# 2235854410/CCVPE

Hardware: AMD Instinct MI355X
Metric: query images/sec (VIGOR, 512x512 sat / 320x640 grd) (higher is better)
Workload: dtype f32; 1 GPU; vigor_samearea_fov360_b32; variant=vigor_ori_prior, batch_per_gpu=32, global_batch=32, parallelism=image-parallel x1, all_gather of 20 B/query results, schedule=two streams per GPU (aerial encoder + orientation decoder on the second)

## Files before the change

ccvpe_amd/_lib.py:

```python
from __future__ import annotations

import ctypes as C
import os

_HERE = os.path.dirname(os.path.abspath(__file__))
LIB_PATH = os.path.join(_HERE, "csrc", "libccvpe_hip.so")

OK = 0
VARIANT_ID = {"vigor": 0, "vigor_ori_prior": 1, "kitti": 2, "oxford": 3}


class Config(C.Structure):
    _fields_ = [("variant", C.c_int32), ("circular_padding", C.c_int32), ("ori_noise", C.c_float),
                ("device", C.c_int32), ("micro_batch", C.c_int32), ("reserved", C.c_int32 * 3)]


class Outputs(C.Structure):
    _fields_ = [("logits_flattened", C.c_void_p), ("heatmap", C.c_void_p), ("ori", C.c_void_p),
                ("matching_score", C.c_void_p * 6)]


class Pose(C.Structure):
    _fields_ = [("index", C.c_int32), ("prob", C.c_float), ("cos_v", C.c_float), ("sin_v", C.c_float),
                ("angle_deg", C.c_float)]


SYMBOLS = [
    ("ccvpe_last_error", C.c_char_p, []),
    ("ccvpe_version", C.c_char_p, []),
    ("ccvpe_launch_count", C.c_uint64, []),
    ("ccvpe_create", C.c_int, [C.POINTER(Config), C.POINTER(C.c_void_p)]),
    ("ccvpe_destroy", C.c_int, [C.c_void_p]),
    ("ccvpe_set_weight", C.c_int, [C.c_void_p, C.c_char_p, C.c_void_p, C.POINTER(C.c_int64), C.c_int32]),
    ("ccvpe_skip_weight", C.c_int, [C.c_void_p, C.c_char_p]),
    ("ccvpe_finalize_weights", C.c_int, [C.c_void_p]),
    ("ccvpe_save_packed", C.c_int, [C.c_void_p, C.c_char_p]),
    ("ccvpe_load_packed", C.c_int, [C.c_void_p, C.c_char_p]),
    ("ccvpe_pack_switches", C.c_char_p, []),
    ("ccvpe_import_tuning", C.c_int, [C.c_void_p, C.c_char_p]),
    ("ccvpe_export_tuning", C.c_int, [C.c_void_p, C.c_char_p, C.c_size_t, C.POINTER(C.c_size_t)]),
    ("ccvpe_tuning_generation", C.c_int, [C.c_void_p]),
    ("ccvpe_max_micro_batch", C.c_int, [C.c_int32, C.c_float, C.c_int32, C.c_int32]),
    ("ccvpe_output_channels", C.c_int, [C.c_void_p, C.c_int32]),
    ("ccvpe_workspace_bytes", C.c_size_t, [C.c_void_p, C.c_int32, C.c_int32, C.c_int32]),
    ("ccvpe_forward", C.c_int, [C.c_void_p, C.c_void_p, C.c_int32, C.c_int32, C.c_void_p, C.c_int32,
                                C.POINTER(Outputs), C.c_void_p]),
    ("ccvpe_postprocess", C.c_int, [C.c_void_p, C.c_void_p, C.c_void_p, C.c_int32, C.c_void_p, C.c_void_p]),
    ("ccvpe_postprocess_rows", C.c_int, [C.c_void_p, C.c_void_p, C.c_void_p, C.c_int32, C.c_void_p, C.c_void_p]),
    ("ccvpe_postprocess_topk", C.c_int, [C.c_void_p, C.c_void_p, C.c_void_p, C.c_int32, C.c_int32, C.c_int32, C.c_void_p,
                                         C.c_void_p]),
    ("ccvpe_eval_metrics", C.c_int, [C.c_void_p, C.c_void_p, C.c_void_p, C.c_int32, C.c_void_p, C.c_void_p, C.c_void_p, C.c_void_p,
                                     C.c_void_p, C.c_void_p]),
    ("ccvpe_aerial_cache_bytes", C.c_size_t, [C.c_void_p, C.c_int32]),
    ("ccvpe_encode_aerial", C.c_int, [C.c_void_p, C.c_void_p, C.c_int32, C.c_void_p, C.c_void_p]),
    ("ccvpe_forward_cached", C.c_int, [C.c_void_p, C.c_void_p, C.c_int32, C.c_int32, C.c_void_p, C.c_int32,
                                       C.POINTER(Outputs), C.c_void_p]),
    ("ccvpe_localize", C.c_int, [C.c_void_p, C.c_void_p, C.c_int32, C.c_int32, C.c_void_p, C.c_int32, C.c_void_p, C.c_void_p]),
    ("ccvpe_localize_cached", C.c_int, [C.c_void_p, C.c_void_p, C.c_int32, C.c_int32, C.c_void_p, C.c_int32, C.c_void_p,
                                        C.c_void_p]),
    ("ccvpe_localize_topk", C.c_int, [C.c_void_p, C.c_void_p, C.c_int32, C.c_int32, C.c_void_p, C.c_int32, C.c_int32, C.c_int32,
                                      C.c_void_p, C.c_void_p]),
    ("ccvpe_localize_topk_cached", C.c_int, [C.c_void_p, C.c_void_p, C.c_int32, C.c_int32, C.c_void_p, C.c_int32, C.c_int32,
                                             C.c_int32, C.c_void_p, C.c_void_p]),
    ("ccvpe_forward_cached_indexed", C.c_int, [C.c_void_p, C.c_void_p, C.c_int32, C.c_int32, C.c_void_p, C.c_int32, C.c_void_p,
                                               C.c_int32, C.POINTER(Outputs), C.c_void_p]),
    ("ccvpe_localize_cached_indexed", C.c_int, [C.c_void_p, C.c_void_p, C.c_int32, C.c_int32, C.c_void_p, C.c_int32, C.c_void_p,
                                                C.c_int32, C.c_void_p, C.c_void_p]),
    ("ccvpe_localize_topk_cached_indexed", C.c_int, [C.c_void_p, C.c_void_p, C.c_int32, C.c_int32, C.c_void_p, C.c_int32, C.c_void_p,
                                                     C.c_int32, C.c_int32, C.c_int32, C.c_void_p, C.c_void_p]),
    ("ccvpe_ground_cache_bytes", C.c_size_t, [C.c_void_p, C.c_int32, C.c_int32, C.c_int32]),
    ("ccvpe_encode_ground", C.c_int, [C.c_void_p, C.c_void_p, C.c_int32, C.c_int32, C.c_int32, C.c_void_p, C.c_void_p]),
    ("ccvpe_localize_region", C.c_int, [C.c_void_p, C.c_void_p, C.c_int32, C.c_int32, C.c_int32, C.c_void_p, C.c_int32, C.c_void_p,
                                        C.c_void_p, C.c_void_p, C.c_void_p, C.c_void_p, C.c_void_p, C.c_void_p, C.c_void_p]),
    ("ccvpe_localize_prior", C.c_int, [C.c_void_p, C.c_void_p, C.c_int32, C.c_int32, C.c_void_p, C.c_int32, C.c_void_p, C.c_int64,
                                       C.c_int32, C.c_int32, C.c_void_p, C.c_void_p]),
    ("ccvpe_localize_prior_cached_indexed", C.c_int, [C.c_void_p, C.c_void_p, C.c_int32, C.c_int32, C.c_void_p, C.c_int32, C.c_void_p,
                                                      C.c_int32, C.c_void_p, C.c_int64, C.c_int32, C.c_int32, C.c_void_p, C.c_void_p]),
    ("ccvpe_postprocess_prior", C.c_int, [C.c_void_p, C.c_void_p, C.c_void_p, C.c_int32, C.c_void_p, C.c_int64, C.c_int32, C.c_int32,
                                          C.c_void_p, C.c_void_p]),
    ("ccvpe_localize_region_prior", C.c_int, [C.c_void_p, C.c_void_p, C.c_int32, C.c_int32, C.c_int32, C.c_void_p, C.c_int32, C.c_void_p,
                                              C.c_void_p, C.c_void_p, C.c_int64, C.c_void_p, C.c_void_p, C.c_void_p, C.c_void_p, C.c_void_p,
                                              C.c_void_p]),
    ("ccvpe_track_update", C.c_int, [C.c_void_p, C.c_void_p, C.c_int32, C.c_int32, C.c_void_p, C.c_int32, C.c_void_p, C.c_int64,
                                     C.c_void_p, C.c_void_p, C.c_void_p]),
    ("ccvpe_track_update_cached_indexed", C.c_int, [C.c_void_p, C.c_void_p, C.c_int32, C.c_int32, C.c_void_p, C.c_int32, C.c_void_p,
                                                    C.c_int32, C.c_void_p, C.c_int64, C.c_void_p, C.c_void_p, C.c_void_p]),
    ("ccvpe_track_update_logits", C.c_int, [C.c_void_p, C.c_void_p, C.c_void_p, C.c_int32, C.c_void_p, C.c_int64, C.c_void_p,
                                            C.c_void_p, C.c_void_p]),
    ("ccvpe_track_predict", C.c_int, [C.c_void_p, C.c_void_p, C.c_int32, C.c_void_p, C.c_void_p, C.c_int32, C.c_int32, C.c_void_p,
                                      C.c_void_p, C.c_void_p]),
    ("ccvpe_preprocess", C.c_int, [C.c_void_p, C.c_int32, C.c_int32, C.c_int32, C.c_void_p, C.c_int32,
                                   C.POINTER(C.c_float * 3), C.POINTER(C.c_float * 3), C.c_void_p, C.c_void_p]),
    ("ccvpe_preprocess_resize", C.c_int, [C.c_void_p, C.c_int32, C.c_int32, C.c_int32, C.c_int32, C.c_int32, C.c_void_p, C.c_int32,
                                          C.POINTER(C.c_float * 3), C.POINTER(C.c_float * 3), C.c_void_p, C.c_void_p, C.c_void_p]),
    ("ccvpe_preprocess_affine", C.c_int, [C.c_void_p, C.c_int32, C.c_int32, C.c_int32, C.c_void_p, C.POINTER(C.c_int32), C.c_int32,
                                          C.c_int32, C.c_int32, C.c_int32, C.c_int32, C.POINTER(C.c_float * 3), C.POINTER(C.c_float * 3),
                                          C.c_void_p, C.c_void_p]),
    ("ccvpe_preprocess_window_resize", C.c_int, [C.c_void_p, C.c_int32, C.c_int32, C.c_void_p, C.c_int32, C.c_int32, C.c_int32,
                                                 C.c_int32, C.c_int32, C.POINTER(C.c_float * 3), C.POINTER(C.c_float * 3), C.c_void_p,
                                                 C.c_void_p, C.c_void_p]),
    ("ccvpe_set_debug", C.c_int, [C.c_void_p, C.c_int32]),
    ("ccvpe_set_streams", C.c_int, [C.c_void_p, C.c_int32]),
    ("ccvpe_read_tap", C.c_int, [C.c_void_p, C.c_char_p, C.c_void_p, C.c_size_t, C.POINTER(C.c_size_t),
                                 C.POINTER(C.c_int32 * 4)]),
    ("ccvpe_debug_dump_plan", C.c_int, [C.c_void_p, C.c_char_p]),
    ("ccvpe_profile_forward", C.c_int, [C.c_void_p, C.c_void_p, C.c_int32, C.c_int32, C.c_void_p, C.c_int32,
                                        C.POINTER(Outputs), C.c_void_p]),
    ("ccvpe_profile_row", C.c_int, [C.c_void_p, C.c_int32, C.c_char_p, C.c_size_t, C.POINTER(C.c_float),
                                    C.POINTER(C.c_double), C.POINTER(C.c_double)]),
    ("ccvpe_profile_row_issued", C.c_int, [C.c_void_p, C.c_int32, C.POINTER(C.c_double)]),
    ("ccvpe_op_num_tiles", C.c_int, []),
    ("ccvpe_op_tile_name", C.c_char_p, [C.c_int32]),
    ("ccvpe_op_conv2d", C.c_int, [C.c_void_p, C.c_int32, C.c_int32, C.c_int32, C.c_int32, C.c_void_p, C.c_void_p,
                                  C.c_int32, C.c_int32, C.c_int32, C.c_int32, C.c_int32, C.c_int32, C.c_int32,
                                  C.c_void_p, C.c_int32, C.POINTER(C.c_float), C.c_void_p]),
]


IMAGENET_MEAN = (0.485, 0.456, 0.406)
IMAGENET_STD = (0.229, 0.224, 0.225)


def preprocess(img_u8_hwc, shift=None, crop_w=None, mean=IMAGENET_MEAN, std=IMAGENET_STD):
    import torch
    lib = load()
    assert img_u8_hwc.is_cuda and img_u8_hwc.dtype == torch.uint8 and img_u8_hwc.dim() == 4 and img_u8_hwc.shape[3] == 3
    img = img_u8_hwc.contiguous()
    B, H, W, _ = img.shape
    crop_w = W if crop_w is None else int(crop_w)
    out = torch.empty((B, 3, H, crop_w), dtype=torch.float32, device=img.device)
    sh = None
    if shift is not None:
        sh = torch.as_tensor(shift, dtype=torch.int32, device=img.device).contiguous()
        assert sh.numel() == B
    m = (C.c_float * 3)(*mean)
    s = (C.c_float * 3)(*std)
    stream = torch.cuda.current_stream(img.device).cuda_stream
    rc = lib.ccvpe_preprocess(C.c_void_p(img.data_ptr()), B, H, W, C.c_void_p(sh.data_ptr()) if sh is not None else None,
                              crop_w, C.byref(m), C.byref(s), C.c_void_p(out.data_ptr()), C.c_void_p(stream))
    check(rc, "ccvpe_preprocess")
    return out


def preprocess_resize(img_u8_hwc, out_hw, shift=None, crop_w=None, mean=IMAGENET_MEAN, std=IMAGENET_STD):
    import torch
    lib = load()
    assert img_u8_hwc.is_cuda and img_u8_hwc.dtype == torch.uint8 and img_u8_hwc.dim() == 4 and img_u8_hwc.shape[3] == 3
    img = img_u8_hwc.contiguous()
    B, H, W, _ = img.shape
    OH, OW = int(out_hw[0]), int(out_hw[1])
    crop_w = OW if crop_w is None else int(crop_w)
    out = torch.empty((B, 3, OH, crop_w), dtype=torch.float32, device=img.device)
    scratch = torch.empty((B, H, OW, 3), dtype=torch.uint8, device=img.device) if W != OW else None
    sh = None
    if shift is not None:
        sh = torch.as_tensor(shift, dtype=torch.int32, device=img.device).contiguous()
        assert sh.numel() == B
    m = (C.c_float * 3)(*mean)
    s = (C.c_float * 3)(*std)
    stream = torch.cuda.current_stream(img.device).cuda_stream
    rc = lib.ccvpe_preprocess_resize(C.c_void_p(img.data_ptr()), B, H, W, OH, OW, C.c_void_p(sh.data_ptr()) if sh is not None else None,
                                     crop_w, C.byref(m), C.byref(s), C.c_void_p(scratch.data_ptr()) if scratch is not None else None,
                                     C.c_void_p(out.data_ptr()), C.c_void_p(stream))
    check(rc, "ccvpe_preprocess_resize")
    return out


RESAMPLE = {"nearest": 0, "bilinear": 2}


def preprocess_affine(img_u8_hwc, matrices, filters, crop, mean=IMAGENET_MEAN, std=IMAGENET_STD):
    import torch
    lib = load()
    assert img_u8_hwc.is_cuda and img_u8_hwc.dtype == torch.uint8 and img_u8_hwc.dim() == 4 and img_u8_hwc.shape[3] == 3
    img = img_u8_hwc.contiguous()
    B, H, W, _ = img.shape
    mat = torch.as_tensor(matrices, dtype=torch.float64).to(img.device).contiguous()
    n = len(filters)
    assert mat.shape == (B, n, 6), (tuple(mat.shape), B, n)
    flt = (C.c_int32 * n)(*[RESAMPLE[f] if isinstance(f, str) else int(f) for f in filters])
    top, left, out_h, out_w = (int(v) for v in crop)
    out = torch.empty((B, 3, max(out_h, 0), max(out_w, 0)), dtype=torch.float32, device=img.device)
    m = (C.c_float * 3)(*mean)
    s = (C.c_float * 3)(*std)
    stream = torch.cuda.current_stream(img.device).cuda_stream
    rc = lib.ccvpe_preprocess_affine(C.c_void_p(img.data_ptr()), B, H, W, C.c_void_p(mat.data_ptr()), flt, n, top, left, out_h, out_w,
                                     C.byref(m), C.byref(s), C.c_void_p(out.data_ptr()), C.c_void_p(stream))
    check(rc, "ccvpe_preprocess_affine")
    return out


def preprocess_window_resize(map_u8_hwc, origins, win_hw, out_hw, mean=IMAGENET_MEAN, std=IMAGENET_STD):
    import torch
    lib = load()
    assert map_u8_hwc.is_cuda and map_u8_hwc.dtype == torch.uint8 and map_u8_hwc.dim() == 3 and map_u8_hwc.shape[2] == 3
    mp = map_u8_hwc.contiguous()
    org = torch.as_tensor(origins, dtype=torch.int32).reshape(-1, 2).to(mp.device).contiguous()
    B = org.shape[0]
    win_h, win_w = int(win_hw[0]), int(win_hw[1])
    out_h, out_w = int(out_hw[0]), int(out_hw[1])
    out = torch.empty((B, 3, max(out_h, 0), max(out_w, 0)), dtype=torch.float32, device=mp.device)
    scratch = torch.empty((max(B * win_h * out_w * 3, 1),), dtype=torch.uint8, device=mp.device)
    m = (C.c_float * 3)(*mean)
    s = (C.c_float * 3)(*std)
    stream = torch.cuda.current_stream(mp.device).cuda_stream
    rc = lib.ccvpe_preprocess_window_resize(C.c_void_p(mp.data_ptr()), mp.shape[0], mp.shape[1], C.c_void_p(org.data_ptr()), B, win_h, win_w,
                                            out_h, out_w, C.byref(m), C.byref(s), C.c_void_p(scratch.data_ptr()), C.c_void_p(out.data_ptr()),
                                            C.c_void_p(stream))
    check(rc, "ccvpe_preprocess_window_resize")
    return out


def op_conv2d(x_nhwc, w, bias=None, stride=1, pad=0, act=0, tile=0, iters=0):
    import torch
    lib = load()
    B, H, W, Cin = x_nhwc.shape
    Cout, _, KH, KW = w.shape
    OH = (H + 2 * pad - KH) // stride + 1
    OW = (W + 2 * pad - KW) // stride + 1
    out = torch.empty((B, OH, OW, Cout), dtype=torch.float32, device=x_nhwc.device)
    x_nhwc = x_nhwc.contiguous()
    w = w.contiguous().float()
    b = bias.contiguous().float() if bias is not None else None
    ms = C.c_float(0.0)
    stream = torch.cuda.current_stream(x_nhwc.device).cuda_stream
    rc = lib.ccvpe_op_conv2d(C.c_void_p(x_nhwc.data_ptr()), B, H, W, Cin, C.c_void_p(w.data_ptr()),
                             C.c_void_p(b.data_ptr()) if b is not None else None, Cout, KH, KW, stride, pad, act, tile,
                             C.c_void_p(out.data_ptr()), iters, C.byref(ms), C.c_void_p(stream))
    check(rc, "ccvpe_op_conv2d")
    return out, (ms.value if iters > 0 else None)

_lib = None


def library_digest() -> str:
    override = os.environ.get("CCVPE_LIB_PATH")
    if override:
        import hashlib
        h = hashlib.sha256()
        with open(override, "rb") as fh:
            for chunk in iter(lambda: fh.read(1 << 20), b""):
                h.update(chunk)
        return h.hexdigest()
    from . import build as _build
    return _build._digest()


def load() -> C.CDLL:
    global _lib
    if _lib is not None:
        return _lib
    try:
        import torch
    except ImportError:
        pass
    override = os.environ.get("CCVPE_LIB_PATH")
    if override:
        lib = C.CDLL(override)
        for name, res, args in SYMBOLS:
            fn = getattr(lib, name)
            fn.restype = res
            fn.argtypes = args
        _lib = lib
        return lib
    try:
        from . import build as _build
        if not _build.is_current():
            _build.build(verbose=False)
    except Exception as e:
        if os.path.exists(LIB_PATH):
            import warnings
            warnings.warn(f"libccvpe_hip.so may be stale and could not be rebuilt: {e}")
    if not os.path.exists(LIB_PATH):
        raise ImportError(
            f"{LIB_PATH} not found: build it with `python -m ccvpe_amd.build` (hipcc, gfx950). "
            "ccvpe_amd has no CPU or PyTorch fallback for the forward pass.")
    lib = C.CDLL(LIB_PATH)
    for name, res, args in SYMBOLS:
        fn = getattr(lib, name)
        fn.restype = res
        fn.argtypes = args
    _lib = lib
    return lib


class CcvpeError(RuntimeError):
    pass


def check(rc: int, what: str) -> None:
    if rc < 0:
        msg = load().ccvpe_last_error()
        raise CcvpeError(f"{what} failed ({rc}): {msg.decode() if msg else ''}")
```

ccvpe_amd/csrc/ccvpe_api.hip:

```cpp
#include "ccvpe_internal.h"

namespace ccvpe { thread_local unsigned long long g_launches = 0; }
static thread_local std::string g_err_storage;
std::string& ccvpe_err() { return g_err_storage; }
int ccvpe_fail(int code, const char* fmt, ...) {
    char buf[1024];
    va_list ap;
    va_start(ap, fmt);
    vsnprintf(buf, sizeof(buf), fmt, ap);
    va_end(ap);
    g_err_storage = buf;
    return code;
}

__global__ __launch_bounds__(256) void checksum_kernel(const uint32_t* __restrict__ p, size_t n, unsigned long long* out) {
    unsigned long long s = 0;
    for (size_t i = (size_t)blockIdx.x * 256 + threadIdx.x; i < n; i += (size_t)gridDim.x * 256) s += (unsigned long long)p[i] * (unsigned long long)((i & 1023) + 1);
    for (int o = 32; o > 0; o >>= 1) s += __shfl_down(s, o);
    if ((threadIdx.x & 63) == 0) atomicAdd(out, s);
}


Switches read_switches() {
    Switches s;
    auto set = [](const char* name) { return getenv(name) != nullptr; };
    auto off = [](const char* name) { const char* e = getenv(name); return e && std::atoi(e) == 0; };
    if (const char* e = getenv("CCVPE_AUTOTUNE")) s.autotune = std::atoi(e) != 0;
    if (const char* e = getenv("CCVPE_FUSE_MBCONV")) s.fuse_mbconv = std::atoi(e);
    if (const char* e = getenv("CCVPE_FUSE_L1")) s.fuse_level1 = std::atoi(e) != 0;
    if (const char* e = getenv("CCVPE_WINOGRAD")) s.wino = std::atoi(e) != 0;
    if (const char* e = getenv("CCVPE_GRAPH")) s.graph_mode = std::atoi(e) != 0;
    if (const char* e = getenv("CCVPE_STREAMS")) s.two_streams = std::atoi(e) >= 2;
    if (const char* e = getenv("CCVPE_PRECISION")) s.precision = (std::string(e) == "bf16x3") ? 1 : 0;
    s.stem_dw = !off("CCVPE_STEM_DW");
    if (const char* e = getenv("CCVPE_FRONT_SPREAD")) s.front_spread = std::atoi(e);
    s.mbconv_image = !off("CCVPE_MBCONV_IMAGE");
    s.se_ticket = !off("CCVPE_SE_TICKET");
    if (const char* e = getenv("CCVPE_SE_PROLOGUE")) s.se_prologue = std::atoi(e) == 1;
    s.split_planes = !set("CCVPE_NO_SPLIT_PLANES");
    s.match_prep_early = !off("CCVPE_MATCH_PREP_EARLY");
    s.match_wide = !off("CCVPE_MATCH_WIDE");
    s.issue_interleaved = !off("CCVPE_ISSUE_ORDER");
    s.log_schedule = set("CCVPE_LOG_SCHEDULE");
    s.no_reuse = set("CCVPE_NO_REUSE");
    s.tune_prefer_pw = set("CCVPE_TUNE_PREFER_PW");
    if (const char* e = getenv("CCVPE_TUNE_PREFER_PROJ")) { s.tune_prefer_proj = true; s.tune_prefer_lat = std::strcmp(e, "lat") == 0; }
    if (const char* e = getenv("CCVPE_TUNE_SPLITK")) s.tune_splitk = std::atoi(e);
    s.tune_no_bf16x3 = set("CCVPE_TUNE_NO_BF16X3");
    s.no_pw = set("CCVPE_NO_PW");
    s.tune_ignore_table = set("CCVPE_TUNE_IGNORE_TABLE");
    s.tune_lat_rows = set("CCVPE_TUNE_LAT_ROWS");
    s.tune_lat_split = set("CCVPE_TUNE_LAT_SPLIT");
    s.tune_no_fused_split = set("CCVPE_TUNE_NO_FUSED_SPLIT");
    if (const char* e = getenv("CCVPE_TUNE_VERBOSE")) s.tune_verbose = e;
    s.no_proj = set("CCVPE_NO_PROJ");
    if (const char* e = getenv("CCVPE_WINO4_MIN_N")) s.wino4_min_n = std::atoi(e);
    s.no_wino4 = set("CCVPE_NO_WINO4");
    s.no_wino4x = set("CCVPE_NO_WINO4X");
    s.pad_concat = !off("CCVPE_PAD_CONCAT");
    if (const char* e = getenv("CCVPE_DIAG_SYNC_BEFORE")) s.diag_sync = e;
    if (const char* e = getenv("CCVPE_DIAG_SNAP")) s.diag_snap = e;
    return s;
}

static int max_micro_batch(const Switches& sw, int variant, float ori_noise, int grd_h, int grd_w) {
    if (variant < 0 || variant > 3) return ccvpe_fail(CCVPE_EINVAL, "unknown variant %d", variant);
    ccvpe_handle_s tmp;
    tmp.cfg.variant = variant; tmp.cfg.ori_noise = ori_noise; tmp.cfg.micro_batch = 1;
    tmp.vs = make_variant(variant);
    tmp.sw = sw;
    tmp.sw.fuse_mbconv = 0; tmp.sw.fuse_level1 = false; tmp.sw.two_streams = false; tmp.sw.graph_mode = 0;
    const int n = (int)(ori_noise / 18.f);
    for (int k = 0; k < 6; ++k) tmp.rolls[k] = (variant == CCVPE_VARIANT_VIGOR_ORI_PRIOR && k > 0) ? 2 * n + 1 : tmp.vs.n_rolls;
    int lo = 0, hi = 1024;
    while (hi - lo > 1) {
        const int mid = (lo + hi) / 2;
        Plan pl;
        PlanKey key;
        key.B = mid; key.gh = grd_h; key.gw = grd_w;
        if (build_plan(&tmp, pl, key) == 0) lo = mid; else hi = mid;
    }
    if (lo == 0) return ccvpe_fail(CCVPE_EINVAL, "ground size %d x %d is not valid for variant %d: %s", grd_h, grd_w, variant, ccvpe_err().c_str());
    return lo;
}

extern "C" {

const char* ccvpe_last_error(void) { return ccvpe_err().c_str(); }
const char* ccvpe_version(void) { return "ccvpe-hip 0.1 (gfx950, fp32 MFMA)"; }
uint64_t ccvpe_launch_count(void) { return ccvpe::g_launches; }

int ccvpe_create(const ccvpe_config* cfg, ccvpe_handle* out) {
    if (!cfg || !out) return ccvpe_fail(CCVPE_EINVAL, "null argument");
    if (cfg->variant < 0 || cfg->variant > 3) return ccvpe_fail(CCVPE_EINVAL, "unknown variant %d", cfg->variant);
    int ndev = 0;
    if (hipGetDeviceCount(&ndev) != hipSuccess || ndev <= 0)
        return ccvpe_fail(CCVPE_EHIP, "no HIP device visible: libccvpe_hip has no CPU fallback");
    if (cfg->device < 0 || cfg->device >= ndev) return ccvpe_fail(CCVPE_EINVAL, "device %d out of range (%d visible)", cfg->device, ndev);
    HIPCHK(hipSetDevice(cfg->device));
    hipDeviceProp_t prop;
    HIPCHK(hipGetDeviceProperties(&prop, cfg->device));
    if (std::string(prop.gcnArchName).find("gfx950") == std::string::npos)
        return ccvpe_fail(CCVPE_EHIP, "device %d is %s; this library carries gfx950 code objects only", cfg->device, prop.gcnArchName);
    auto* h = new ccvpe_handle_s();
    h->cfg = *cfg;
    if (h->cfg.micro_batch <= 0) h->cfg.micro_batch = 32;
    h->vs = make_variant(cfg->variant);
    h->sw = read_switches();
    if (h->sw.precision) h->cfg.reserved[0] = *h->sw.precision;
    if (h->cfg.reserved[0] != 0 && h->cfg.reserved[0] != 1) { delete h; return ccvpe_fail(CCVPE_EINVAL, "unknown precision mode %d", cfg->reserved[0]); }
    const int n = (int)(cfg->ori_noise / 18.f);
    for (int k = 0; k < 6; ++k)
        h->rolls[k] = (cfg->variant == CCVPE_VARIANT_VIGOR_ORI_PRIOR && k > 0) ? 2 * n + 1 : h->vs.n_rolls;
    if (cfg->variant == CCVPE_VARIANT_VIGOR_ORI_PRIOR && (n < 0 || 2 * n + 1 > 32)) {
        delete h;
        return ccvpe_fail(CCVPE_EINVAL, "ori_noise %.1f out of range", cfg->ori_noise);
    }
    build_expect(h);
    *out = h;
    return 0;
}

int ccvpe_max_micro_batch(int32_t variant, float ori_noise, int32_t grd_h, int32_t grd_w) {
    return max_micro_batch(read_switches(), variant, ori_noise, grd_h, grd_w);
}

int ccvpe_destroy(ccvpe_handle h) {
    if (!h) return 0;
    (void)hipSetDevice(h->cfg.device);
    for (void* p : h->dev_allocs) (void)hipFree(p);
    if (h->arena) (void)hipFree(h->arena);
    for (auto* buf : {&h->post_scratch, &h->topk_scratch, &h->prior_scratch}) if (buf->ptr) (void)hipFree(buf->ptr);
    h->plans.clear();
    for (int k = 0; k < 2; ++k) if (h->snap[k]) (void)hipFree(h->snap[k]);
    if (h->capture_stream) (void)hipStreamDestroy(h->capture_stream);
    if (h->aux_stream) (void)hipStreamDestroy(h->aux_stream);
    delete h;
    return 0;
}

int ccvpe_output_channels(ccvpe_handle h, int32_t level) {
    if (!h || level < 0 || level > 5) return ccvpe_fail(CCVPE_EINVAL, "bad level");
    return h->rolls[level];
}

size_t ccvpe_workspace_bytes(ccvpe_handle h, int32_t batch, int32_t grd_h, int32_t grd_w) {
    if (!h || !h->finalized || batch <= 0) { ccvpe_fail(CCVPE_ESTATE, "handle not ready"); return 0; }
    Plan pl;
    PlanKey key;
    key.B = std::min(batch, h->cfg.micro_batch); key.gh = grd_h; key.gw = grd_w;
    if (build_plan(h, pl, key)) return 0;
    return pl.total * sizeof(float);
}

}

static void check_issued_tile(Plan& pl, const Op& op) {
    const int got = conv_tile_last();
    if (!op.tile || (*op.tile & 0xff) == 0 || got == 0) return;
    const int want = *op.tile, ws = (want >> 8) & 0xff, gs = (got >> 8) & 0xff;
    if ((want & 0xff) != (got & 0xff) || (ws > 1 ? ws : 1) != (gs > 1 ? gs : 1))
        std::fprintf(stderr, "ccvpe: launch %s (batch %d) runs %s split %d instead of the planned %s split %d\n", op.name.c_str(), pl.key.B,
                     conv_tile_name(got), gs, conv_tile_name(want), ws);
}

static int run_ops(ccvpe_handle h, Plan& pl, const Ctx& base, hipStream_t s0) {
    const bool check = !pl.tiles_checked;
    pl.tiles_checked = true;
    if (check) (void)conv_tile_last();
    if (!pl.two_streams || h->serial_issue) {
        Ctx c = base;
        c.stream = s0;
        for (auto& op : pl.ops) { op.fn(c); if (check) check_issued_tile(pl, op); }
        base.conv_errors += c.conv_errors;
        return 0;
    }
    if (!h->aux_stream) HIPCHK(hipStreamCreateWithFlags(&h->aux_stream, hipStreamNonBlocking));
    if (pl.events.empty()) {
        pl.events.assign(pl.ops.size() + 2, nullptr);
        for (size_t i = 0; i < pl.events.size(); ++i)
            if (i >= pl.ops.size() || pl.ops[i].signal) HIPCHK(hipEventCreateWithFlags(&pl.events[i], hipEventDisableTiming));
    }
// ... 781 lines not shown
    }
    if (n_bil > WARP_MAX_BILINEAR) return ccvpe_fail(CCVPE_EINVAL, "%d BILINEAR stages (at most %d)", n_bil, WARP_MAX_BILINEAR);
    if (batch <= 0 || batch > 65535) return ccvpe_fail(CCVPE_EINVAL, "batch %d out of range (1..65535)", batch);
    if (H <= 0 || W <= 0 || H > 16384 || W > 16384) return ccvpe_fail(CCVPE_EINVAL, "canvas %d x %d out of range (1..16384 per side)", H, W);
    if (out_h <= 0 || out_w <= 0 || top < 0 || left < 0 || top > H - out_h || left > W - out_w)
        return ccvpe_fail(CCVPE_EINVAL, "crop (top %d, left %d, %d x %d) outside the %d x %d canvas", top, left, out_h, out_w, H, W);
    WarpParams p{};
    p.in = hwc; p.mat = matrices; p.B = batch; p.H = H; p.W = W; p.n = n_stages; p.bilinear = bil;
    p.top = top; p.left = left; p.out_h = out_h; p.out_w = out_w; p.out = out_nchw;
    for (int c = 0; c < 3; ++c) { p.mean[c] = mean[c]; p.stdv[c] = stdv[c]; }
    if (launch_warp(p, (hipStream_t)stream) != 0) return ccvpe_fail(CCVPE_EINVAL, "no kernel for this stage pattern");
    return launch_status("affine launch");
}

int ccvpe_preprocess_window_resize(const uint8_t* map_hwc, int32_t map_h, int32_t map_w, const int32_t* origins, int32_t batch,
                                   int32_t win_h, int32_t win_w, int32_t out_h, int32_t out_w, const float mean[3], const float stdv[3],
                                   uint8_t* scratch, float* out_nchw, void* stream) {
    if (!map_hwc || !origins || !mean || !stdv || !scratch || !out_nchw) return ccvpe_fail(CCVPE_EINVAL, "null argument");
    if (map_h <= 0 || map_w <= 0 || batch <= 0 || win_h <= 0 || win_w <= 0 || out_h <= 0 || out_w <= 0) return ccvpe_fail(CCVPE_EINVAL, "bad geometry");
    if (win_w > 8 * out_w || win_h > 8 * out_h)
        return ccvpe_fail(CCVPE_EINVAL, "down-scaling factors above 8 are not supported (%dx%d -> %dx%d)", win_h, win_w, out_h, out_w);
    if ((double)batch * win_h * out_w * 3 >= 2147483647.0 * 2 || (double)batch * 3 * out_h * out_w >= 2147483647.0 * 2)
        return ccvpe_fail(CCVPE_EINVAL, "window batch too large");
    ResizeParams p{};
    p.in = map_hwc; p.B = batch; p.IH = win_h; p.IW = win_w; p.OH = out_h; p.OW = out_w; p.crop_w = out_w; p.tmp = scratch; p.out = out_nchw;
    p.origin = origins; p.map_h = map_h; p.map_w = map_w;
    for (int c = 0; c < 3; ++c) { p.mean[c] = mean[c]; p.stdv[c] = stdv[c]; }
    if (launch_resize(p, (hipStream_t)stream) != 0) return ccvpe_fail(CCVPE_EINVAL, "down-scaling factors above 8 are not supported");
    return launch_status("window resize launch");
}

int ccvpe_debug_dump_plan(ccvpe_handle h, const char* path) {
    if (!h || !path) return ccvpe_fail(CCVPE_EINVAL, "null argument");
    Plan* pl = h->last_plan;
    if (!pl) return ccvpe_fail(CCVPE_ESTATE, "no forward has run on this handle");
    HIPCHK(hipSetDevice(h->cfg.device));
    HIPCHK(hipDeviceSynchronize());
    const size_t n = pl->size.size();
    unsigned long long* d = nullptr;
    HIPCHK(hipMalloc((void**)&d, n * sizeof(unsigned long long)));
    HIPCHK(hipMemset(d, 0, n * sizeof(unsigned long long)));
    for (size_t id = 0; id < n; ++id) {
        if (pl->size[id] == 0) continue;
        const int blocks = (int)std::min<size_t>((pl->size[id] + 255) / 256, 2048);
        CCVPE_LAUNCH(checksum_kernel, dim3(blocks), dim3(256), 0, nullptr, reinterpret_cast<const uint32_t*>(h->arena + pl->off[id]), pl->size[id], d + id);
    }
    std::vector<unsigned long long> sums(n);
    hipError_t e = hipMemcpy(sums.data(), d, n * sizeof(unsigned long long), hipMemcpyDeviceToHost);
    (void)hipFree(d);
    if (e != hipSuccess) return ccvpe_fail(CCVPE_EHIP, "checksum copy failed: %s", hipGetErrorString(e));
    FILE* f = std::fopen(path, "w");
    if (!f) return ccvpe_fail(CCVPE_EINVAL, "cannot open %s", path);
    std::fprintf(f, "# plan B=%d grd=%dx%d mode=%d two_streams=%d tensors=%zu arena_floats=%zu\n", pl->key.B, pl->key.gh, pl->key.gw, pl->key.mode, (int)pl->two_streams, n, pl->total);
    for (size_t i = 0; i < pl->ops.size(); ++i) {
        const Op& op = pl->ops[i];
        std::fprintf(f, "op %zu %s stream=%d wait=%d signal=%d tile=%s", i, op.name.c_str(), op.stream, op.wait_on.empty() ? -1 : op.wait_on[0], (int)op.signal,
                     op.tile ? conv_tile_name(*op.tile) : "-");
        if (op.tile && (*op.tile >> 8) == 255) std::fprintf(f, "_tailsplit");
        else if (op.tile && (*op.tile >> 8) > SPLIT_FUSED) std::fprintf(f, "_splitk%dr", (*op.tile >> 8) - SPLIT_FUSED);
        else if (op.tile && (*op.tile >> 8) > 1) std::fprintf(f, "_splitk%d", *op.tile >> 8);
        for (int id : op.uses) std::fprintf(f, " t%d[off=%zu,n=%zu]=%016llx", id, pl->off[id], pl->size[id], sums[id]);
        std::fprintf(f, "\n");
    }
    if (h->snap[0]) {
        for (int which = 0; which < 2; ++which) {
            std::fprintf(f, "snap_%s %s", which ? "after" : "before", h->sw.diag_snap.c_str());
            for (auto& e : h->snap_layout) {
                unsigned long long* dd = nullptr;
                unsigned long long v = 0;
                if (hipMalloc((void**)&dd, sizeof(v)) == hipSuccess) {
                    (void)hipMemset(dd, 0, sizeof(v));
                    const int blocks = (int)std::min<size_t>((pl->size[e.first] + 255) / 256, 2048);
                    CCVPE_LAUNCH(checksum_kernel, dim3(blocks), dim3(256), 0, nullptr, reinterpret_cast<const uint32_t*>(h->snap[which] + e.second), pl->size[e.first], dd);
                    (void)hipMemcpy(&v, dd, sizeof(v), hipMemcpyDeviceToHost);
                    (void)hipFree(dd);
                }
                std::fprintf(f, " t%d=%016llx", e.first, v);
            }
            std::fprintf(f, "\n");
        }
    }
    std::fclose(f);
    return 0;
}

int ccvpe_op_num_tiles(void) { return conv_num_tiles(); }
const char* ccvpe_op_tile_name(int32_t tile) { return conv_tile_name(tile); }

int ccvpe_op_conv2d(const float* in, int32_t B, int32_t H, int32_t W, int32_t Cin, const float* w, const float* bias,
                    int32_t Cout, int32_t KH, int32_t KW, int32_t stride, int32_t pad, int32_t act, int32_t tile,
                    float* out, int32_t iters, float* ms, void* stream) {
    if (!in || !w || !out) return ccvpe_fail(CCVPE_EINVAL, "null argument");
    if (B <= 0 || H <= 0 || W <= 0 || Cin <= 0 || Cin % 8 || Cout <= 0 || KH <= 0 || KW <= 0 || stride <= 0 || pad < 0)
        return ccvpe_fail(CCVPE_EINVAL, "bad conv geometry (Cin must be a multiple of 8)");
    const int OH = (H + 2 * pad - KH) / stride + 1, OW = (W + 2 * pad - KW) / stride + 1;
    if (OH <= 0 || OW <= 0) return ccvpe_fail(CCVPE_EINVAL, "empty output");
    if ((double)B * H * W * Cin >= 2147483647.0 || (double)B * OH * OW * Cout >= 2147483647.0)
        return ccvpe_fail(CCVPE_EINVAL, "tensor exceeds 2^31 elements");
    const size_t nw = (size_t)Cout * Cin * KH * KW;
    std::vector<float> hw(nw), hb(Cout, 0.f);
    HIPCHK(hipMemcpy(hw.data(), w, nw * sizeof(float), hipMemcpyDefault));
    if (bias) HIPCHK(hipMemcpy(hb.data(), bias, Cout * sizeof(float), hipMemcpyDefault));
    ccvpe_handle_s tmp;
    tmp.sw = read_switches();
    tmp.cfg.reserved[0] = 1;
    PackedConv pc;
    const int taps = KH * KW;
    int rc = pack_conv(&tmp, pc, Cout, taps, Cin, Cin, identity_map(Cin),
                       [&](int n, int t, int c) { return hw[((size_t)n * Cin + c) * taps + t]; }, hb, KH, KW);
    auto cleanup = [&]() { for (void* p : tmp.dev_allocs) (void)hipFree(p); };
    if (rc) { cleanup(); return rc; }
    ConvParams p = conv_params(pc, in, Cin, B, H, W, OH, OW, stride, pad, pad, act);
    p.dst[0] = {out, Cout, 0}; p.ndst = 1;
    hipStream_t st = (hipStream_t)stream;
    if (((tile >> 8) & 0xff) > 1) {
        int sk = (tile >> 8) & 0xff;
        if (sk > SPLIT_FUSED && sk != 255) sk -= SPLIT_FUSED;
        {
            void* d = nullptr;
            if (hipMalloc(&d, CONV_TICKETS * sizeof(unsigned)) != hipSuccess || hipMemset(d, 0, CONV_TICKETS * sizeof(unsigned)) != hipSuccess) { cleanup(); return ccvpe_fail(CCVPE_ENOMEM, "ticket counters"); }
            tmp.dev_allocs.push_back(d);
            tmp.dev_alloc_bytes.push_back(CONV_TICKETS * sizeof(unsigned));
            p.tickets = (unsigned*)d;
        }
        const size_t fl = (size_t)(sk == 255 ? 8 : sk) * p.M * p.N;
        void* d = nullptr;
        if (hipMalloc(&d, fl * sizeof(float)) != hipSuccess) { cleanup(); return ccvpe_fail(CCVPE_ENOMEM, "split-K slab"); }
        tmp.dev_allocs.push_back(d);
        tmp.dev_alloc_bytes.push_back(fl * sizeof(float));
        p.partial = (float*)d; p.partial_floats = fl;
    }
    if (const ConvTile* t = conv_tile(tile); t && t->family == TILE_WINO && !conv_tile_runs(*t, p)) { cleanup(); return ccvpe_fail(CCVPE_EINVAL, "layer is not Winograd-shaped (3x3, stride 1, pad 1, W %% 16 == 0, H %% 16 == 0, output channels a multiple of 4; F(4x4): >= 40 of them)"); }
    if (launch_conv_igemm(p, tile, st) != 0) { cleanup(); return ccvpe_fail(CCVPE_EINVAL, "unsupported conv geometry (KH*KW <= 16, Cin %% 8 == 0)"); }
    hipError_t e = hipGetLastError();
    if (e == hipSuccess && iters > 0 && ms) {
        hipEvent_t e0, e1;
        (void)hipEventCreate(&e0); (void)hipEventCreate(&e1);
        (void)hipEventRecord(e0, st);
        for (int i = 0; i < iters; ++i) launch_conv_igemm(p, tile, st);
        (void)hipEventRecord(e1, st);
        (void)hipEventSynchronize(e1);
        float t = 0.f;
        (void)hipEventElapsedTime(&t, e0, e1);
        *ms = t / iters;
        (void)hipEventDestroy(e0); (void)hipEventDestroy(e1);
    }
    hipError_t e2 = hipStreamSynchronize(st);
    cleanup();
    if (e != hipSuccess) return ccvpe_fail(CCVPE_EHIP, "conv launch failed: %s", hipGetErrorString(e));
    if (e2 != hipSuccess) return ccvpe_fail(CCVPE_EHIP, "conv execution failed: %s", hipGetErrorString(e2));
    return 0;
}

}
```

ccvpe_amd/csrc/ccvpe_internal.h:

```cpp
#pragma once
#include "../../include/ccvpe.h"
#include "kernels.h"

#include <algorithm>
#include <cmath>
#include <cstdarg>
#include <cstdio>
#include <cstdlib>
#include <cstring>
#include <functional>
#include <map>
#include <memory>
#include <optional>
#include <set>
#include <string>
#include <type_traits>
#include <vector>

using namespace ccvpe;

std::string& ccvpe_err();
int ccvpe_fail(int code, const char* fmt, ...);
#define HIPCHK(expr)                                                                           \
    do {                                                                                       \
        hipError_t _e = (expr);                                                                \
        if (_e != hipSuccess) return ccvpe_fail(CCVPE_EHIP, "%s failed: %s", #expr, hipGetErrorString(_e)); \
    } while (0)

struct BlockSpec { int e, k, s, cin, cout; };
static const BlockSpec B0[16] = {
    {1, 3, 1, 32, 16}, {6, 3, 2, 16, 24}, {6, 3, 1, 24, 24}, {6, 5, 2, 24, 40}, {6, 5, 1, 40, 40},
    {6, 3, 2, 40, 80}, {6, 3, 1, 80, 80}, {6, 3, 1, 80, 80}, {6, 5, 1, 80, 112}, {6, 5, 1, 112, 112},
    {6, 5, 1, 112, 112}, {6, 5, 2, 112, 192}, {6, 5, 1, 192, 192}, {6, 5, 1, 192, 192}, {6, 5, 1, 192, 192},
    {6, 3, 1, 192, 320},
};
static const int TAP_BLOCK[5] = {15, 10, 4, 2, 0};
static const float BN_EPS = 1e-3f;

struct DecLevel { int din, dout, skip, mid, out; };
struct VariantSpec {
    int feat_h;
    int head_ch[6];
    int sat_desc;
    int match_ch[6];
    int step[6];
    int n_rolls;
    int centre;
    DecLevel loc[6], ori[6];
};
static const DecLevel VIGOR_LOC[6] = {{1281, 1024, 320, 640, 640}, {641, 320, 112, 320, 320}, {321, 160, 40, 160, 160},
                                      {161, 80, 24, 80, 80},       {81, 40, 16, 40, 40},      {41, 16, 0, 16, 1}};
static const DecLevel VIGOR_ORI[6] = {{1300, 1024, 320, 640, 640}, {640, 256, 112, 256, 256}, {256, 128, 40, 128, 128},
                                      {128, 64, 24, 64, 64},       {64, 32, 16, 32, 32},      {32, 16, 0, 16, 2}};
static const DecLevel KITTI_LOC[6] = {{2049, 1024, 320, 512, 512}, {513, 256, 112, 256, 256}, {257, 128, 40, 128, 128},
                                      {129, 64, 24, 128, 128},     {129, 32, 16, 32, 32},     {33, 16, 0, 16, 1}};
static const DecLevel KITTI_ORI[6] = {{2064, 1024, 320, 512, 512}, {512, 256, 112, 256, 256}, {256, 128, 40, 128, 128},
                                      {128, 64, 24, 64, 64},       {64, 32, 16, 32, 32},      {32, 16, 0, 16, 2}};

static VariantSpec make_variant(int v) {
    VariantSpec s{};
    auto cp = [](DecLevel* d, const DecLevel* src) { for (int i = 0; i < 6; ++i) d[i] = src[i]; };
    if (v == CCVPE_VARIANT_KITTI) {
        s.feat_h = 8;
        int hc[6] = {16, 8, 4, 2, 1, 1}, mc[6] = {2048, 512, 256, 128, 128, 32}, st[6] = {128, 64, 32, 16, 8, 8};
        for (int i = 0; i < 6; ++i) { s.head_ch[i] = hc[i]; s.match_ch[i] = mc[i]; s.step[i] = st[i]; }
        s.sat_desc = 2048; s.n_rolls = 16; s.centre = 0;
        cp(s.loc, KITTI_LOC); cp(s.ori, KITTI_ORI);
    } else {
        int mc[6] = {1280, 640, 320, 160, 80, 40}, st[6] = {64, 32, 16, 8, 4, 2};
        int hv[6] = {64, 32, 16, 8, 4, 2}, ho[6] = {32, 16, 8, 4, 2, 1};
        for (int i = 0; i < 6; ++i) {
            s.match_ch[i] = mc[i]; s.step[i] = st[i];
            s.head_ch[i] = (v == CCVPE_VARIANT_OXFORD) ? ho[i] : hv[i];
        }
        s.feat_h = (v == CCVPE_VARIANT_OXFORD) ? 4 : 10;
        s.sat_desc = 1280; s.n_rolls = 20; s.centre = (v == CCVPE_VARIANT_OXFORD);
        cp(s.loc, VIGOR_LOC); cp(s.ori, VIGOR_ORI);
    }
    return s;
}

static void static_pad(int k, int s, int& lo, int& hi) {
    if (s == 1) { lo = hi = (k - 1) / 2; return; }
    int total = k - 2;
    lo = total / 2; hi = total - lo;
}
static int conv_out(int n, int k, int s) {
    int lo, hi; static_pad(k, s, lo, hi);
    return (n + lo + hi - k) / s + 1;
}
static int se_squeeze(int cin) { return std::max(1, (int)(cin * 0.25)); }
static int round_up(int a, int b) { return (a + b - 1) / b * b; }
static int deconv_width(const DecLevel& l, bool pad) {
    return (pad && l.skip > 0 && (l.dout * 4) % 64 != 0) ? round_up(l.dout, 16) : l.dout;
}

struct Switches {
    bool autotune = true;
    int fuse_mbconv = 1;
    bool fuse_level1 = true;
    bool wino = true;
    int graph_mode = 0;
    bool two_streams = true;
    std::optional<int> precision;
    bool stem_dw = true;
    std::optional<int> front_spread;
    bool mbconv_image = true;
    bool se_ticket = true;
    bool se_prologue = false;
    bool split_planes = true;
    bool match_prep_early = true;
    bool match_wide = true;
    bool issue_interleaved = true;
    bool log_schedule = false;
    bool no_reuse = false;
    bool tune_prefer_pw = false;
    bool tune_prefer_proj = false;
    bool tune_prefer_lat = false;
    std::optional<int> tune_splitk;
    bool tune_no_bf16x3 = false;
    bool no_pw = false;
    bool tune_ignore_table = false;
    bool tune_lat_rows = false;
    bool tune_lat_split = false;
    bool tune_no_fused_split = false;
    std::string tune_verbose;
    bool no_proj = false;
    int wino4_min_n = 40;
    bool no_wino4 = false;
    bool no_wino4x = false;
    bool pad_concat = true;
    std::string diag_sync, diag_snap;

    bool tune_filtered() const {
        return tune_prefer_pw || tune_prefer_proj || tune_splitk || tune_no_bf16x3 || no_pw || tune_ignore_table || tune_lat_rows || tune_lat_split ||
               tune_no_fused_split;
    }
    std::string pack_group() const {
        std::string s;
        if (no_proj) s += "CCVPE_NO_PROJ=1;";
        if (wino4_min_n != 40) s += "CCVPE_WINO4_MIN_N=" + std::to_string(wino4_min_n) + ";";
        if (no_wino4) s += "CCVPE_NO_WINO4=1;";
        if (no_wino4x) s += "CCVPE_NO_WINO4X=1;";
        if (!pad_concat) s += "CCVPE_PAD_CONCAT=0;";
        return s;
    }
};
Switches read_switches();

struct PackedConv {
    float* w = nullptr;
    unsigned short *w_hi = nullptr, *w_lo = nullptr;
    float* bias = nullptr;
    int N = 0, Kpad = 0, nchunks = 0, cinp = 0, KH = 1, KW = 1;
    float* wino = nullptr;
    int wino_n16 = 0;
    size_t wino_bytes = 0;
    float* wino4 = nullptr;
    size_t wino4_bytes = 0;
    float* wino4x = nullptr;
    size_t wino4x_bytes = 0;
    int wino4x_cfg = -1;
    float* proj = nullptr;
    size_t proj_bytes = 0;
};
struct BlockW {
    PackedConv expand, project;
    float* exp_lin = nullptr;
    int exp_cinp = 0;
    float *dw_w = nullptr, *dw_b = nullptr, *se_w1 = nullptr, *se_b1 = nullptr, *se_w2 = nullptr, *se_b2 = nullptr;
    int sq = 0;
};
struct EncoderW {
    float *stem_w = nullptr, *stem_b = nullptr;
    BlockW blk[16];
    PackedConv head;
};
struct DecoderW {
    PackedConv deconv[6], conva[6], convb[5];
    float* tail_w = nullptr;
    float* l1_wt = nullptr;
    float tail_b[2] = {0.f, 0.f};
    float *l1_wc = nullptr, *l1_ws = nullptr, *l1_bc = nullptr;
    int l1_cx = 0, l1_cxp = 0, l1_c0 = 0, l1_ng = 0, l1_score = 0;
};

struct Tensor {
    int id = -1; int B = 0, H = 0, W = 0, C = 0;
    bool split = false;
    long long numel() const { return (long long)B * H * W * C; }
};

struct Ctx {
    float* arena = nullptr;
    const std::vector<size_t>* off = nullptr;
    hipStream_t stream = nullptr;
    const float* grd = nullptr;
    const float* sat = nullptr;
    ccvpe_outputs out{};
    float* splitk_scratch = nullptr;
    size_t splitk_floats = 0;
    unsigned* tickets = nullptr;
    const float* cache_in = nullptr;
    float* cache_out = nullptr;
    float* rows = nullptr;
    int topk_k = 0, topk_r = 0;
    const int* tile_index = nullptr;
    int n_tiles = 0;
    const float* grd_cache_in = nullptr;
    const int* query_index = nullptr;
    int n_queries = 0;
    float* stats = nullptr;
    const float* log_prior = nullptr;
    long long prior_stride = 0;
    float* posterior = nullptr;
    float* ptr(const Tensor& t) const { return arena + (*off)[t.id]; }
    Dst dst(const Tensor& t, int coff = 0) const { return Dst{ptr(t), t.C, coff, t.split ? 1 : 0, t.numel()}; }
    mutable int conv_errors = 0;
    mutable size_t conv_tick_off = 0;
    mutable ConvParams* probe = nullptr;
    void launch_conv(ConvParams& p, int cfg) const {
        p.tickets = tickets ? tickets + conv_tick_off : nullptr;
        p.partial = splitk_scratch;
        p.partial_floats = splitk_floats;
        if (probe) { *probe = p; return; }
        if (launch_conv_igemm(p, cfg, stream) != 0) ++conv_errors;
    }
};

struct PlanKey {
    int B = 0, gh = 0, gw = 0;
    int mode = 0;
    bool pose = false;
    bool topk = false;
    bool operator==(const PlanKey& o) const { return B == o.B && gh == o.gh && gw == o.gw && mode == o.mode && pose == o.pose && topk == o.topk; }
};

struct ForwardCall {
    const float* grd = nullptr;
    int gh = 0, gw = 0;
    const float* sat = nullptr;
    const float* cache = nullptr;
    const int32_t* tile_index = nullptr;
    int n_tiles = 0;
    int batch = 0;
    const ccvpe_outputs* out = nullptr;
    float* rows = nullptr;
    int topk_k = 0, topk_r = 0;
    const float* log_prior = nullptr;
    long long prior_stride = 0;
    float* posterior = nullptr;
    hipStream_t stream = nullptr;
    bool profile = false;
    PlanKey plan_key() const {
        PlanKey key;
        key.gh = gh; key.gw = gw; key.mode = cache ? 2 : 0; key.pose = rows != nullptr; key.topk = rows && topk_k > 0;
        return key;
    }
};

struct Op {
    std::string name;
    std::function<void(const Ctx&)> fn;
    std::vector<int> uses;
    double flops = 0, bytes = 0;
    std::shared_ptr<int> tile;
    int gemm_m = 0, gemm_n = 0, gemm_kpad = 0;
    int conv_cin = 0;
    bool bf16x3_only = false;
    bool wino_ok = false;
    bool wino4_ok = false;
    bool wino4x_ok = false;
    bool is_pw = false;
    bool proj_ok = false;
    int stream = 0;
    std::vector<int> wait_on;
    bool signal = false;
};

struct TapInfo { Tensor t; int coff; int C; };

struct Plan {
    PlanKey key;
    bool debug = false;
    std::vector<size_t> size;
    std::vector<size_t> off;
    std::vector<Op> ops;
    std::map<std::string, TapInfo> taps;
    size_t total = 0;
    float* arena = nullptr;
    Tensor scratch;
    bool use_graph = false;
    Tensor io_grd, io_sat, io_logits, io_heat, io_ori, io_ms[6];
    Tensor tune_cache;
    hipGraphExec_t exec = nullptr;
    int runs = 0;
    size_t ticket_words = 0;
    unsigned* tickets = nullptr;
    size_t alloc_tickets(size_t n) { const size_t o = ticket_words; ticket_words += (n + 15) & ~(size_t)15; return o; }
    bool tiles_checked = false;
    bool two_streams = false;
    Tensor scratch2;
    std::vector<hipEvent_t> events;
    std::vector<int> issue_order;
    bool issue_interleaved = true, log_schedule = false, no_reuse = false;
    ~Plan() {
        if (exec) (void)hipGraphExecDestroy(exec);
        for (hipEvent_t e : events) if (e) (void)hipEventDestroy(e);
        if (tickets) (void)hipFree(tickets);
    }
    void schedule() {
        if (!two_streams) return;
        bool any = false;
        for (auto& o : ops) {
            o.stream = (o.name.rfind("sat.", 0) == 0 || o.name.rfind("ori", 0) == 0) ? 1 : 0;
            any = any || o.stream == 1;
            o.wait_on.clear();
            o.signal = false;
        }
        if (!any) { two_streams = false; return; }
        std::map<int, int> last_use;
        for (int i = 0; i < (int)ops.size(); ++i) {
            int dep = -1;
            for (int id : ops[i].uses) {
                auto it = last_use.find(id);
                if (it != last_use.end() && ops[it->second].stream != ops[i].stream) dep = std::max(dep, it->second);
            }
            if (dep >= 0) { ops[i].wait_on.push_back(dep); ops[dep].signal = true; }
            for (int id : ops[i].uses) last_use[id] = i;
        }
        issue_order.clear();
        {
            std::vector<int> q[2];
            for (int i = 0; i < (int)ops.size(); ++i) q[ops[i].stream].push_back(i);
            size_t p[2] = {0, 0};
            std::vector<bool> issued(ops.size(), false);
            while (issue_interleaved && (p[0] < q[0].size() || p[1] < q[1].size())) {
                auto ready = [&](int s) {
// ... 158 lines not shown
```

ccvpe_amd/csrc/ccvpe_plan.hip:

```cpp
#include "ccvpe_internal.h"

static int window_offset(const VariantSpec& vs, int level, int L) {
    const int C = vs.match_ch[level];
    return vs.centre ? (int)((double)C / 2 - (double)L / 2) : 0;
}
static int mod(int a, int m) { int r = a % m; return r < 0 ? r + m : r; }

ConvParams conv_params(const PackedConv& pc, const float* in, int in_ld, int B, int H, int W, int OH, int OW,
                              int stride, int pad_t, int pad_l, int act) {
    ConvParams p{};
    p.in = in; p.in_ld = in_ld; p.B = B; p.H = H; p.W = W; p.Cin = pc.cinp; p.OH = OH; p.OW = OW;
    p.KH = pc.KH; p.KW = pc.KW; p.stride = stride; p.pad_t = pad_t; p.pad_l = pad_l;
    p.wpk = pc.w; p.w_hi = pc.w_hi; p.w_lo = pc.w_lo; p.Kpad = pc.Kpad; p.Npad = round_up(pc.N, conv_igemm_npad()); p.nchunks = pc.nchunks; p.bias = pc.bias; p.N = pc.N; p.act = act;
    p.gate = nullptr; p.resid = nullptr; p.resid_ld = 0; p.ndst = 0; p.mode = MODE_CONV; p.deconv_cout = 0;
    p.M = B * OH * OW;
    p.in_bytes = (unsigned)((size_t)B * H * W * in_ld * sizeof(float));
    p.gate_bytes = (unsigned)((size_t)B * pc.cinp * sizeof(float));
    p.w_plane_bytes = (unsigned)((size_t)p.Npad * pc.Kpad * sizeof(unsigned short));
    p.wino_w = pc.wino; p.wino_n16 = pc.wino_n16; p.wino_bytes = (unsigned)pc.wino_bytes;
    p.wino4_w = pc.wino4; p.wino4_bytes = (unsigned)pc.wino4_bytes;
    p.wino4x_w = pc.wino4x; p.wino4x_bytes = (unsigned)pc.wino4x_bytes; p.wino4x_cfg = pc.wino4x_cfg;
    p.proj_w = pc.proj; p.proj_bytes = (unsigned)pc.proj_bytes;
    return p;
}
// ... 258 lines not shown
    pl.two_streams = h->sw.two_streams && !h->debug;
    pl.issue_interleaved = h->sw.issue_interleaved; pl.log_schedule = h->sw.log_schedule; pl.no_reuse = h->sw.no_reuse;
    if (pl.two_streams) pl.scratch2 = pl.alloc(1, 1, 1, (int)Plan::SPLITK_FLOATS);
    pl.use_graph = !cached && !pose && h->sw.graph_mode == 1;
    if (pl.use_graph) {
        pl.io_grd = pl.alloc(B, 3, gh, gw);
        pl.io_sat = pl.alloc(B, 3, CCVPE_SAT_HW, CCVPE_SAT_HW);
        pl.io_logits = pl.alloc(B, 1, CCVPE_OUT_HW, CCVPE_OUT_HW);
        pl.io_heat = pl.alloc(B, 1, CCVPE_OUT_HW, CCVPE_OUT_HW);
        pl.io_ori = pl.alloc(B, 2, CCVPE_OUT_HW, CCVPE_OUT_HW);
        for (int k = 0; k < 6; ++k) pl.io_ms[k] = pl.alloc(B, h->rolls[k], 8 << k, 8 << k);
    }

    int fh, fw, L[6];
    if (int rc = grd_geometry(vs, gh, gw, fh, fw, L)) return rc;

    const int D = vs.sat_desc;
    const int rfull = vs.n_rolls;
    const int rpad = score_pad(rfull);
    Tensor loc_in[6], ori_in6;
    Tensor loc_cat[6], ori_cat[6];
    for (int j = 0; j < 6; ++j) {
        const int hw_in = 8 << j;
        loc_in[j] = pl.alloc(B, hw_in, hw_in, 8 + vs.match_ch[j]);
        loc_cat[j] = pl.alloc(B, hw_in * 2, hw_in * 2, deconv_width(vs.loc[j], h->sw.pad_concat) + vs.loc[j].skip);
        ori_cat[j] = pl.alloc(B, hw_in * 2, hw_in * 2, deconv_width(vs.ori[j], h->sw.pad_concat) + vs.ori[j].skip);
        if (h->cfg.reserved[0] == 1 && j < 5 && h->sw.split_planes) { loc_cat[j].split = true; ori_cat[j].split = true; }
    }
    ori_in6 = pl.alloc(B, 8, 8, rpad + D);
    pl.taps["ori_in6"] = {ori_in6, 0, ori_in6.C};

    EncOut genc, senc;
    if (!grd_cached) plan_encoder(h, pl, h->grd_enc, true, B, gh, gw, h->cfg.circular_padding != 0, nullptr, genc, "grd");
    TapDst td[5];
    for (int t = 0; t < 5; ++t) {
        td[t].n = 2;
        td[t].t[0] = loc_cat[t]; td[t].coff[0] = deconv_width(vs.loc[t], h->sw.pad_concat);
        td[t].t[1] = ori_cat[t]; td[t].coff[1] = deconv_width(vs.ori[t], h->sw.pad_concat);
    }
    size_t coff[6];
    cache_layout(vs, B, coff);
    if (!cached) {
        plan_encoder(h, pl, h->sat_enc, false, B, CCVPE_SAT_HW, CCVPE_SAT_HW, false, td, senc, "sat");
    } else {
        size_t one[6];
        cache_layout(vs, 1, one);
        for (int t = 0; t < 5; ++t) {
            Tensor lc = loc_cat[t], oc = ori_cat[t];
            const int lcoff = deconv_width(vs.loc[t], h->sw.pad_concat), ocoff = deconv_width(vs.ori[t], h->sw.pad_concat);
            const size_t src_off = coff[t + 1], src_off1 = one[t + 1];
            const int C = TAP_C[t], hw = TAP_HW[t];
            const long long P = (long long)B * TAP_HW[t];
            pl.add("sat.cached_tap" + std::to_string(TAP_BLOCK[t]), {lc, oc}, [=](const Ctx& c) {
                if (c.tile_index)
                    launch_gather_channels(c.cache_in + src_off1 * c.n_tiles, C, hw, c.tile_index, B, c.dst(lc, lcoff), c.dst(oc, ocoff), 2, c.stream);
                else
                    launch_scatter_channels(c.cache_in + src_off, C, P, c.dst(lc, lcoff), c.dst(oc, ocoff), 2, c.stream);
            }, 0, 4.0 * P * C * 3);
        }
    }

    int ltot = 0, loff[6];
    for (int k = 0; k < 6; ++k) { loff[k] = ltot; ltot += round_up(L[k], 4); }
    Tensor desc;
    if (grd_cached) {
        desc = pl.alloc(B, 1, 1, ltot);
        Tensor d = desc;
        pl.add("grd.cached_desc", {d}, [=](const Ctx& c) {
            launch_gather_channels(c.grd_cache_in, ltot, 1, c.query_index, B, c.dst(d), Dst{nullptr, 0, 0, 0, 0}, 1, c.stream);
        }, 0, 8.0 * B * ltot);
    } else {
        desc = plan_grd_desc(h, pl, B, fh, fw, genc.vol, false);
    }
    for (int k = 0; k < 6; ++k) pl.taps["grd_desc" + std::to_string(k + 1)] = {desc, loff[k], L[k]};

    Tensor dmap = pl.alloc(B, 8, 8, D);
    if (cached) {
        Tensor dm = dmap;
        const long long P = (long long)B * 64;
        pl.add("sat.cached_descmap", {dm}, [=](const Ctx& c) {
            if (c.tile_index)
                launch_gather_channels(c.cache_in, D, 64, c.tile_index, B, c.dst(dm), Dst{nullptr, 0, 0, 0, 0}, 1, c.stream);
            else
                launch_scatter_channels(c.cache_in, D, P, c.dst(dm), Dst{nullptr, 0, 0, 0, 0}, 1, c.stream);
        }, 0, 8.0 * P * D);
        pl.taps["sat_descriptor_map"] = {dmap, 0, D};
    } else {
        const PackedConv* pc = &h->sat_desc;
        Tensor x = senc.vol;
        pl.add_conv("sat.descmap", {x, dmap}, B * 8 * 8, pc->N, pc->Kpad, [=](const Ctx& c, int tile) {
            ConvParams p = conv_params(*pc, c.ptr(x), 1280, B, 16, 16, 8, 8, 2, 0, 0, ACT_NONE);
            p.dst[0] = {c.ptr(dmap), D, 0}; p.ndst = 1;
            c.launch_conv(p, tile);
        }, 2.0 * B * 64 * 5120.0 * D, 4.0 * (B * 256 * 1280.0 + 5120.0 * D));
        pl.ops.back().proj_ok = pc->proj != nullptr && h->cfg.reserved[0] == 0;
        pl.taps["sat_descriptor_map"] = {dmap, 0, D};
    }

    auto plan_level = [&](const DecoderW& dw, const DecLevel* lv, int j, Tensor din, Tensor cat, const std::string& tag) -> Tensor {
        const int hin = 8 << j, hout = hin * 2;
        const DecLevel& l = lv[j];
        {
            const PackedConv* pc = &dw.deconv[j];
            const int cout = deconv_width(l, h->sw.pad_concat);
            pl.add_conv(tag + ".deconv", {din, cat}, B * hin * hin, pc->N, pc->Kpad, [=](const Ctx& c, int tile) {
                ConvParams p = conv_params(*pc, c.ptr(din), din.C, B, hin, hin, hin, hin, 1, 0, 0, ACT_NONE);
                p.mode = MODE_DECONV; p.deconv_cout = cout;
                p.dst[0] = c.dst(cat); p.ndst = 1;
                c.launch_conv(p, tile);
            }, 2.0 * B * hin * hin * (double)l.din * 4 * l.dout, 4.0 * B * hin * hin * ((double)din.C + 4.0 * l.dout));
            pl.ops.back().is_pw = !din.split;
            pl.ops.back().proj_ok = pc->proj != nullptr && !din.split && h->cfg.reserved[0] == 0;
        }
        Tensor mid = pl.alloc(B, hout, hout, l.mid);
        mid.split = cat.split;
        {
            const PackedConv* pc = &dw.conva[j];
            pl.add_conv(tag + ".conv_a", {cat, mid}, B * hout * hout, pc->N, pc->Kpad, [=](const Ctx& c, int tile) {
                ConvParams p = conv_params(*pc, c.ptr(cat), cat.C, B, hout, hout, hout, hout, 1, 1, 1, ACT_RELU);
                p.in_split = cat.split; p.in_plane_bytes = (unsigned)(cat.numel() * 2);
                p.dst[0] = c.dst(mid); p.ndst = 1;
                c.launch_conv(p, tile);
            }, 2.0 * B * hout * hout * 9.0 * cat.C * l.mid, 4.0 * B * hout * hout * ((double)cat.C + l.mid));
            pl.ops.back().bf16x3_only = cat.split;
            pl.ops.back().conv_cin = cat.C;
            pl.ops.back().wino_ok = pc->wino != nullptr && !cat.split && h->sw.wino && h->cfg.reserved[0] == 0;
            pl.ops.back().wino4_ok = pl.ops.back().wino_ok && pc->wino4 != nullptr;
            pl.ops.back().wino4x_ok = pl.ops.back().wino_ok && pc->wino4x != nullptr;
        }
        if (j == 5) return mid;
        Tensor o = pl.alloc(B, hout, hout, l.out);
        {
            const PackedConv* pc = &dw.convb[j];
            pl.add_conv(tag + ".conv_b", {mid, o}, B * hout * hout, pc->N, pc->Kpad, [=](const Ctx& c, int tile) {
                ConvParams p = conv_params(*pc, c.ptr(mid), mid.C, B, hout, hout, hout, hout, 1, 1, 1, ACT_NONE);
                p.in_split = mid.split; p.in_plane_bytes = (unsigned)(mid.numel() * 2);
                p.dst[0] = {c.ptr(o), o.C, 0}; p.ndst = 1;
                c.launch_conv(p, tile);
            }, 2.0 * B * hout * hout * 9.0 * l.mid * l.out, 4.0 * B * hout * hout * ((double)l.mid + l.out));
            pl.ops.back().bf16x3_only = mid.split;
            pl.ops.back().conv_cin = mid.C;
            pl.ops.back().wino_ok = pc->wino != nullptr && !mid.split && h->sw.wino && h->cfg.reserved[0] == 0;
            pl.ops.back().wino4_ok = pl.ops.back().wino_ok && pc->wino4 != nullptr;
            pl.ops.back().wino4x_ok = pl.ops.back().wino_ok && pc->wino4x != nullptr;
        }
        return o;
    };

    auto plan_level1_fused = [&](const DecoderW& dw, Tensor din, int cin_real, int cout, bool is_ori, Tensor raw, const std::string& tag, Tensor out_ws = Tensor{}) {
        Level1Params lp{};
        lp.x_ld = din.C; lp.cx = dw.l1_cx; lp.cxp = dw.l1_cxp; lp.B = B; lp.H = CCVPE_OUT_HW; lp.W = CCVPE_OUT_HW;
        lp.c0 = dw.l1_c0; lp.ng = dw.l1_ng; lp.score = dw.l1_score; lp.wc = dw.l1_wc; lp.ws = dw.l1_ws; lp.bc = dw.l1_bc; lp.wt = dw.l1_wt;
        lp.bt[0] = dw.tail_b[0]; lp.bt[1] = dw.tail_b[1]; lp.cout = cout; lp.normalize = is_ori ? 1 : 0;
        const bool has_raw = raw.id >= 0;
        std::vector<Tensor> uses = {din};
        if (has_raw) uses.push_back(raw);
        if (out_ws.id >= 0) uses.push_back(out_ws);
        const double px = (double)B * CCVPE_OUT_HW * CCVPE_OUT_HW;
        pl.add(tag + ".fused", uses, [=](const Ctx& c) {
            Level1Params q = lp;
            q.x = c.ptr(din);
            q.out = out_ws.id >= 0 ? c.ptr(out_ws) : is_ori ? c.out.ori : c.out.logits_flattened;
            q.raw = has_raw ? c.ptr(raw) : nullptr;
            launch_level1(q, c.stream);
        }, px / 4 * 2.0 * cin_real * 64 + px * 2.0 * 144 * 16 + px * 2.0 * 144 * cout, 4.0 * (px / 4 * lp.cx + px * cout));
    };

    Tensor x = dmap;
    Tensor loc_mid;
    const Tensor logits_ws = pose ? pl.alloc(B, 1, CCVPE_OUT_HW, CCVPE_OUT_HW) : Tensor{};
    const bool prep_early = h->sw.match_prep_early;
    size_t first_match_op = (size_t)-1;
    std::vector<std::function<MatchParams(const Ctx&)>> prep_fills;
    std::vector<Tensor> prep_uses;
    for (int k = 0; k < 6; ++k) {
        MatchParams mp{};
        const int hw = (8 << k) * (8 << k);
        const int C = vs.match_ch[k];
        mp.x_ld = x.C; mp.B = B; mp.HW = hw; mp.C = C; mp.g_ld = ltot; mp.L = L[k];
        const int off = window_offset(vs, k, L[k]);
        const bool prior = h->cfg.variant == CCVPE_VARIANT_VIGOR_ORI_PRIOR;
        const int n = prior ? (int)(h->cfg.ori_noise / 18.f) : 0;
        if (k == 0 || !prior) {
            mp.R = rfull;
            for (int r = 0; r < rfull; ++r) mp.shift[r] = mod(off + r * vs.step[k], C);
            mp.inmax = 0;
            if (prior) { for (int i = -n; i <= n; ++i) mp.inmax |= 1u << mod(i, rfull); }
            else mp.inmax = rfull >= 32 ? 0xffffffffu : ((1u << rfull) - 1u);
        } else {
            mp.R = 2 * n + 1;
            for (int r = 0; r < mp.R; ++r) mp.shift[r] = mod(off + (r - n) * vs.step[k], C);
            mp.inmax = (mp.R >= 32) ? 0xffffffffu : ((1u << mp.R) - 1u);
        }
        mp.rpad = rpad;
        mp.P = match_pixels_per_block(hw, C);
        mp.no_wide = h->sw.match_wide ? 0 : 1;
        mp.cat_max_ld = 8 + C;
        mp.cat_all_ld = rpad + C;
        Tensor xin = x, lin = loc_in[k];
        Tensor ggs = pl.alloc(B, 1, 1, (int)match_scratch_floats(C));
        const bool first = (k == 0);
        const int goff = loff[k];
        const int R = mp.R;
        std::vector<Tensor> uses = {xin, desc, lin, ggs};
        if (first) uses.push_back(ori_in6);
        mp.prep_done = prep_early ? 1 : 0;
        auto fill = [=](const Ctx& c) {
            MatchParams q = mp;
            q.x = c.ptr(xin); q.g = c.ptr(desc) + goff;
            q.ms = pose ? nullptr : c.out.matching_score[k];
            q.cat_max = c.ptr(lin);
            q.cat_all = first ? c.ptr(ori_in6) : nullptr;
            q.gg_scratch = c.ptr(ggs);
            return q;
        };
        if (first_match_op == (size_t)-1) first_match_op = pl.ops.size();
        if (prep_early) {
            prep_fills.push_back(fill);
            if (prep_uses.empty()) prep_uses.push_back(desc);
            prep_uses.push_back(ggs);
        }
        pl.add("match" + std::to_string(k + 1), uses, [=](const Ctx& c) { launch_match(fill(c), c.stream); },
               4.0 * B * hw * (double)R * L[k], 4.0 * B * hw * (2.0 * C + R + 8));
        pl.taps["loc_in" + std::to_string(6 - k)] = {lin, 0, lin.C};
        if (k == 5 && h->sw.fuse_level1) { plan_level1_fused(h->loc, lin, vs.loc[5].din, 1, false, Tensor{}, "loc1", logits_ws); break; }
        Tensor o = plan_level(h->loc, vs.loc, k, lin, loc_cat[k], "loc" + std::to_string(6 - k));
        if (k < 5) { pl.taps["loc_level" + std::to_string(6 - k)] = {o, 0, o.C}; x = o; }
        else loc_mid = o;
    }
    if (!prep_fills.empty()) {
        const size_t n0 = pl.ops.size();
        pl.add("match.prep", prep_uses, [prep_fills](const Ctx& c) {
            MatchParams ps[6];
            const int n = (int)std::min<size_t>(prep_fills.size(), 6);
            for (int i = 0; i < n; ++i) ps[i] = prep_fills[i](c);
            launch_match_prep_all(ps, n, c.stream);
        }, 0.0, 0.0);
        std::rotate(pl.ops.begin() + first_match_op, pl.ops.begin() + n0, pl.ops.end());
    }
    if (!h->sw.fuse_level1) {
        Tensor m = loc_mid;
        const float* tw = h->loc.tail_w;
        const float tb = h->loc.tail_b[0];
        std::vector<Tensor> uses = {m};
        if (pose) uses.push_back(logits_ws);
        pl.add("loc1.tail", uses, [=](const Ctx& c) {
            TailConvParams p{};
            p.in = c.ptr(m); p.B = B; p.H = CCVPE_OUT_HW; p.W = CCVPE_OUT_HW; p.w = tw; p.bias[0] = tb; p.cout = 1;
            p.normalize = 0; p.out = pose ? c.ptr(logits_ws) : c.out.logits_flattened; p.raw = nullptr;
            launch_tail_conv(p, c.stream);
        }, 2.0 * B * 262144.0 * 144, 4.0 * B * 262144.0 * 17);
    }
    Tensor pose_index;
    if (pose) {
        static_assert(CCVPE_OUT_HW * CCVPE_OUT_HW == 64 * 4096, "pose_argmax_kernel: 64 chunks of 4096 values");
        const bool topk = pl.key.topk;
        Tensor part = pl.alloc(B, 1, 64, 2), keys = pl.alloc(B, 1, 64, topk ? 2 * TOPK_MAX_K : 2);
        pose_index = pl.alloc(B, 1, 1, topk ? TOPK_MAX_K : 1);
        const Tensor lg = logits_ws, idx = pose_index;
        pl.add("softmax.partial", {lg, part}, [=](const Ctx& c) {
            SoftmaxParams p{};
            p.logits = c.ptr(lg); p.B = B; p.n = CCVPE_OUT_HW * CCVPE_OUT_HW; p.partial = c.ptr(part); p.chunks = 64; p.out = nullptr;
            p.prior = c.log_prior; p.prior_stride = c.prior_stride;
            launch_softmax_partial(p, c.stream);
        }, 0, 4.0 * B * 262144.0);
        const size_t toff = pl.alloc_tickets((size_t)B);
        if (topk) pl.add("topk.peaks", {lg, part, keys, idx}, [=](const Ctx& c) {
            TopkParams p{};
            p.heat = nullptr; p.logits = c.ptr(lg); p.partial = c.ptr(part); p.B = B; p.k = c.topk_k; p.r = c.topk_r;
            p.keys = reinterpret_cast<unsigned long long*>(c.ptr(keys)); p.tickets = c.tickets + toff;
            p.index = reinterpret_cast<int*>(c.ptr(idx)); p.rows = c.rows;
            p.prior = c.log_prior; p.prior_stride = c.prior_stride;
            launch_topk_peaks(p, c.stream);
        }, 0, 4.0 * B * 262144.0);
        else pl.add("pose.argmax", {lg, part, keys, idx}, [=](const Ctx& c) {
            PoseArgmaxParams p{};
            p.logits = c.ptr(lg); p.partial = c.ptr(part); p.B = B; p.n = CCVPE_OUT_HW * CCVPE_OUT_HW; p.chunks = 64;
            p.pairs = c.ptr(keys); p.tickets = c.tickets + toff; p.index = reinterpret_cast<int*>(c.ptr(idx)); p.rows = c.rows;
            p.stats = c.stats; p.prior = c.log_prior; p.prior_stride = c.prior_stride; p.posterior = c.posterior;
            launch_pose_argmax(p, c.stream);
        }, 0, 4.0 * B * 262144.0);
    } else {
        Tensor part = pl.alloc(B, 1, 64, 2);
        pl.add("softmax", {part}, [=](const Ctx& c) {
            SoftmaxParams p{};
            p.logits = c.out.logits_flattened; p.B = B; p.n = CCVPE_OUT_HW * CCVPE_OUT_HW; p.partial = c.ptr(part); p.chunks = 64;
            p.out = c.out.heatmap;
            launch_softmax(p, c.stream);
        }, 0, 4.0 * B * 262144.0 * 3);
    }
    {
        Tensor xo = ori_in6;
        Tensor ori_mid;
        Tensor raw;
        if (h->debug && !pose) { raw = pl.alloc(B, 2, CCVPE_OUT_HW, CCVPE_OUT_HW); pl.taps["ori_level1_nchw"] = {raw, 0, -1}; }
        bool fused_done = false;
        for (int j = 0; j < 6; ++j) {
            if (j == 5 && h->sw.fuse_level1 && pose) {
                const DecoderW& dw = h->ori;
                Level1Params lp{};
                lp.x_ld = xo.C; lp.cx = dw.l1_cx; lp.cxp = dw.l1_cxp; lp.B = B; lp.H = CCVPE_OUT_HW; lp.W = CCVPE_OUT_HW;
                lp.c0 = dw.l1_c0; lp.ng = dw.l1_ng; lp.score = dw.l1_score; lp.wc = dw.l1_wc; lp.ws = dw.l1_ws; lp.bc = dw.l1_bc; lp.wt = dw.l1_wt;
                lp.bt[0] = dw.tail_b[0]; lp.bt[1] = dw.tail_b[1]; lp.cout = 2; lp.normalize = 1;
                const Tensor din = xo, idx = pose_index;
                const bool topk = pl.key.topk;
                const double px = (double)B * (topk ? 8 : 1) * 16 * 16, cin_real = vs.ori[5].din;
// ... 108 lines not shown
```

ccvpe_amd/csrc/ccvpe_weights.hip:

```cpp
#include "ccvpe_internal.h"

#include <unistd.h>

static void add_bn(std::map<std::string, std::vector<int64_t>>& m, const std::string& p, int c) {
    m[p + ".weight"] = {c}; m[p + ".bias"] = {c}; m[p + ".running_mean"] = {c}; m[p + ".running_var"] = {c};
    m[p + ".num_batches_tracked"] = {};
}
static void add_encoder(std::map<std::string, std::vector<int64_t>>& m, const std::string& p) {
    m[p + "._conv_stem.weight"] = {32, 3, 3, 3};
    add_bn(m, p + "._bn0", 32);
    for (int i = 0; i < 16; ++i) {
        const BlockSpec& b = B0[i];
        std::string q = p + "._blocks." + std::to_string(i);
        int mid = b.cin * b.e;
        if (b.e != 1) { m[q + "._expand_conv.weight"] = {mid, b.cin, 1, 1}; add_bn(m, q + "._bn0", mid); }
        m[q + "._depthwise_conv.weight"] = {mid, 1, b.k, b.k};
        add_bn(m, q + "._bn1", mid);
        int sq = se_squeeze(b.cin);
        m[q + "._se_reduce.weight"] = {sq, mid, 1, 1}; m[q + "._se_reduce.bias"] = {sq};
        m[q + "._se_expand.weight"] = {mid, sq, 1, 1}; m[q + "._se_expand.bias"] = {mid};
        m[q + "._project_conv.weight"] = {b.cout, mid, 1, 1};
        add_bn(m, q + "._bn2", b.cout);
    }
    m[p + "._conv_head.weight"] = {1280, 320, 1, 1};
// ... 28 lines not shown
}

static int upload(ccvpe_handle_s* h, const std::vector<float>& v, float** out) {
    void* d = nullptr;
    size_t bytes = std::max<size_t>(v.size(), 4) * sizeof(float);
    HIPCHK(hipMalloc(&d, bytes));
    h->dev_allocs.push_back(d);
    h->dev_alloc_bytes.push_back(bytes);
    HIPCHK(hipMemcpy(d, v.data(), v.size() * sizeof(float), hipMemcpyHostToDevice));
    *out = (float*)d;
    return 0;
}

extern "C" const char* ccvpe_pack_switches(void) {
    static thread_local std::string s;
    s = read_switches().pack_group();
    return s.c_str();
}

int pack_conv(ccvpe_handle_s* h, PackedConv& pc, int N, int taps, int cin, int cinp, const std::vector<int>& cmap,
                     const std::function<float(int, int, int)>& get, const std::vector<float>& bias, int KH, int KW) {
    const int npad = round_up(N, conv_igemm_npad());
    const int K = taps * cinp;
    const int kpad = round_up(K, 32);
    std::vector<float> w((size_t)npad * kpad, 0.f);
    for (int n = 0; n < N; ++n)
        for (int t = 0; t < taps; ++t)
            for (int c = 0; c < cin; ++c) w[(size_t)n * kpad + conv_igemm_k_index(cinp, taps, t, cmap[c])] = get(n, t, c);
    pc.N = N; pc.Kpad = kpad; pc.nchunks = K / 8; pc.cinp = cinp; pc.KH = KH; pc.KW = KW;
    int rc = upload(h, w, &pc.w);
    if (rc) return rc;
    if (((KH == 1 && KW == 1 && taps == 1 && cin == cinp && conv_proj_wanted(N, cin)) || conv_proj_lat_wanted(taps, KH, KW, cinp)) && !h->sw.no_proj) {
        std::vector<int> inv(cinp, -1);
        for (int c = 0; c < cin; ++c) inv[cmap[c]] = c;
        std::vector<float> up;
        conv_proj_pack(N, cinp, [&](int n, int k) { const int t = k / cinp, c = inv[k - t * cinp]; return c >= 0 ? get(n, t, c) : 0.f; }, up, taps);
        pc.proj_bytes = up.size() * sizeof(float);
        if ((rc = upload(h, up, &pc.proj))) return rc;
    }
    if (KH == 3 && KW == 3 && cin == cinp && cin % 8 == 0 && (size_t)(cin / 8) * 16 * ((N + 15) / 16) * 512 < (1u << 31)) {
        std::vector<float> u;
        conv_wino_pack(N, cin, get, u, &pc.wino_n16);
        pc.wino_bytes = u.size() * sizeof(float);
        if ((rc = upload(h, u, &pc.wino))) return rc;
        if (N >= h->sw.wino4_min_n && (size_t)((cin + 15) / 16) * 4 * 9 * ((N + 15) / 16) * 1024 < (1u << 31) && !h->sw.no_wino4) {
            std::vector<float> u4;
            conv_wino4_pack(N, cin, get, u4);
            pc.wino4_bytes = u4.size() * sizeof(float);
            if ((rc = upload(h, u4, &pc.wino4))) return rc;
        }
        if (N >= 24 && conv_wino4x_config(N) >= 0 && !h->sw.no_wino4x) {
            std::vector<float> ux;
            conv_wino4x_pack(N, cin, get, ux, &pc.wino4x_cfg);
            pc.wino4x_bytes = ux.size() * sizeof(float);
            if ((rc = upload(h, ux, &pc.wino4x))) return rc;
        }
    }
    if (h->cfg.reserved[0] == 1) {
        auto to_bf16 = [](float f) -> unsigned short {
            uint32_t u; std::memcpy(&u, &f, 4);
            if ((u & 0x7fffffffu) > 0x7f800000u) return (unsigned short)((u >> 16) | 0x40);
            return (unsigned short)((u + 0x7fffu + ((u >> 16) & 1u)) >> 16);
        };
        std::vector<unsigned short> hi(w.size()), lo(w.size());
        for (size_t i = 0; i < w.size(); ++i) {
            hi[i] = to_bf16(w[i]);
            uint32_t hu = (uint32_t)hi[i] << 16; float hf; std::memcpy(&hf, &hu, 4);
            lo[i] = to_bf16(w[i] - hf);
        }
        for (int plane = 0; plane < 2; ++plane) {
            void* d = nullptr;
            HIPCHK(hipMalloc(&d, hi.size() * sizeof(unsigned short)));
            h->dev_allocs.push_back(d);
            h->dev_alloc_bytes.push_back(hi.size() * sizeof(unsigned short));
            HIPCHK(hipMemcpy(d, plane ? lo.data() : hi.data(), hi.size() * sizeof(unsigned short), hipMemcpyHostToDevice));
            (plane ? pc.w_lo : pc.w_hi) = (unsigned short*)d;
        }
    }
    return upload(h, bias, &pc.bias);
}
std::vector<int> identity_map(int n) { std::vector<int> m(n); for (int i = 0; i < n; ++i) m[i] = i; return m; }

struct BnFold { std::vector<float> scale, shift; };
static BnFold fold_bn(ccvpe_handle_s* h, const std::string& p) {
    const auto& g = h->host[p + ".weight"]; const auto& b = h->host[p + ".bias"];
    const auto& mu = h->host[p + ".running_mean"]; const auto& var = h->host[p + ".running_var"];
    BnFold f; f.scale.resize(g.size()); f.shift.resize(g.size());
    for (size_t i = 0; i < g.size(); ++i) {
        float s = g[i] / std::sqrt(var[i] + BN_EPS);
        f.scale[i] = s; f.shift[i] = b[i] - mu[i] * s;
    }
    return f;
}

static int pack_pointwise_bn(ccvpe_handle_s* h, PackedConv& pc, const std::string& wkey, const std::string& bnkey, int cout, int cin) {
    const auto& w = h->host[wkey];
    BnFold f = fold_bn(h, bnkey);
    return pack_conv(h, pc, cout, 1, cin, cin, identity_map(cin),
                     [&](int n, int, int c) { return w[(size_t)n * cin + c] * f.scale[n]; }, f.shift, 1, 1);
}

static int build_encoder(ccvpe_handle_s* h, EncoderW& e, const std::string& p) {
    int rc;
    {
        const auto& w = h->host[p + "._conv_stem.weight"];
        BnFold f = fold_bn(h, p + "._bn0");
        std::vector<float> pk(27 * 32);
        for (int o = 0; o < 32; ++o)
            for (int k = 0; k < 27; ++k) pk[k * 32 + o] = w[o * 27 + k] * f.scale[o];
        if ((rc = upload(h, pk, &e.stem_w))) return rc;
        if ((rc = upload(h, f.shift, &e.stem_b))) return rc;
    }
    for (int i = 0; i < 16; ++i) {
        const BlockSpec& b = B0[i];
        BlockW& bw = e.blk[i];
        std::string q = p + "._blocks." + std::to_string(i);
        const int mid = b.cin * b.e;
        if (b.e != 1 && (rc = pack_pointwise_bn(h, bw.expand, q + "._expand_conv.weight", q + "._bn0", mid, b.cin))) return rc;
        if (b.e != 1 && (mbconv_front_supported(b.k, b.s, b.cin, mid) || b.cin % 8 == 0)) {
            const auto& w = h->host[q + "._expand_conv.weight"];
            BnFold f = fold_bn(h, q + "._bn0");
            bw.exp_cinp = round_up(b.cin, 16);
            std::vector<float> lin((size_t)mid * bw.exp_cinp, 0.f);
            for (int n = 0; n < mid; ++n)
                for (int c = 0; c < b.cin; ++c) lin[(size_t)n * bw.exp_cinp + c] = w[(size_t)n * b.cin + c] * f.scale[n];
            if ((rc = upload(h, lin, &bw.exp_lin))) return rc;
        }
        {
            const auto& w = h->host[q + "._depthwise_conv.weight"];
            BnFold f = fold_bn(h, q + "._bn1");
            const int kk = b.k * b.k;
            std::vector<float> pk((size_t)kk * mid);
            for (int c = 0; c < mid; ++c)
                for (int t = 0; t < kk; ++t) pk[(size_t)t * mid + c] = w[(size_t)c * kk + t] * f.scale[c];
            if ((rc = upload(h, pk, &bw.dw_w))) return rc;
            if ((rc = upload(h, f.shift, &bw.dw_b))) return rc;
        }
        bw.sq = se_squeeze(b.cin);
        if ((rc = upload(h, h->host[q + "._se_reduce.weight"], &bw.se_w1))) return rc;
        if ((rc = upload(h, h->host[q + "._se_reduce.bias"], &bw.se_b1))) return rc;
        {
            const auto& w2 = h->host[q + "._se_expand.weight"];
            std::vector<float> t((size_t)mid * bw.sq);
            for (int c = 0; c < mid; ++c)
                for (int j = 0; j < bw.sq; ++j) t[(size_t)j * mid + c] = w2[(size_t)c * bw.sq + j];
            if ((rc = upload(h, t, &bw.se_w2))) return rc;
        }
        if ((rc = upload(h, h->host[q + "._se_expand.bias"], &bw.se_b2))) return rc;
        if ((rc = pack_pointwise_bn(h, bw.project, q + "._project_conv.weight", q + "._bn2", b.cout, mid))) return rc;
    }
    return pack_pointwise_bn(h, e.head, p + "._conv_head.weight", p + "._bn1", 1280, 320);
}


static int build_decoder(ccvpe_handle_s* h, DecoderW& d, const DecLevel* lv, const std::string& sfx, int nscore_l6, bool every_level_scored) {
    int rc;
    for (int j = 0; j < 6; ++j) {
        std::string n = std::to_string(6 - j);
        {
            const auto& w = h->host["deconv" + n + sfx + ".weight"];
            const auto& b = h->host["deconv" + n + sfx + ".bias"];
            const int cin = lv[j].din, cout = lv[j].dout, cw = deconv_width(lv[j], h->sw.pad_concat);
            int nscore = 0;
            if (every_level_scored) nscore = 1;
            else if (j == 0) nscore = nscore_l6;
            const int spad = score_pad(nscore);
            const int cinp = spad + (cin - nscore);
            std::vector<int> cmap(cin);
            for (int c = 0; c < cin; ++c) cmap[c] = c < nscore ? c : c - nscore + spad;
            std::vector<float> bias(4 * cw, 0.f);
            for (int qd = 0; qd < 4; ++qd) for (int o = 0; o < cout; ++o) bias[qd * cw + o] = b[o];
            if ((rc = pack_conv(h, d.deconv[j], 4 * cw, 1, cin, cinp, cmap,
                                [&](int nn, int, int c) { int qd = nn / cw, o = nn % cw; return o < cout ? w[((size_t)c * cout + o) * 4 + qd] : 0.f; },
                                bias, 1, 1))) return rc;
        }
        if (j == 5) {
            const auto& w = h->host["deconv" + n + sfx + ".weight"];
            const auto& b = h->host["deconv" + n + sfx + ".bias"];
            const auto& wa = h->host["conv" + n + sfx + ".0.weight"];
            const auto& ba = h->host["conv" + n + sfx + ".0.bias"];
            const int cin = lv[j].din, cout = lv[j].dout;
            const int nscore = every_level_scored ? 1 : 0;
            const int spad = score_pad(nscore);
            const int cd = cin - nscore;
            d.l1_cx = spad + cd;
            d.l1_cxp = round_up(d.l1_cx, 16);
            d.l1_c0 = spad; d.l1_ng = (cd + 3) / 4; d.l1_score = nscore;
            std::vector<double> wc((size_t)16 * cin * 16, 0.0);
            for (int py = 0; py < 2; ++py)
                for (int px = 0; px < 2; ++px)
                    for (int ky = 0; ky < 3; ++ky)
                        for (int kx = 0; kx < 3; ++kx) {
                            const int ty = py + ky + 1, tx = px + kx + 1, a = (ty >> 1) - py, bb = (tx >> 1) - px;
                            const int qd = (ty & 1) * 2 + (tx & 1);
                            double* dst = &wc[(size_t)(((py * 2 + px) * 2 + a) * 2 + bb) * cin * 16];
                            for (int c = 0; c < cin; ++c)
                                for (int o = 0; o < 16; ++o) {
                                    double acc = 0.0;
                                    for (int m = 0; m < cout; ++m)
                                        acc += (double)wa[((size_t)o * 16 + m) * 9 + ky * 3 + kx] * (double)w[((size_t)c * cout + m) * 4 + qd];
                                    dst[(size_t)c * 16 + o] += acc;
                                }
                        }
            std::vector<float> pk((size_t)4 * d.l1_ng * 64 * 4, 0.f), sc(4 * 64, 0.f);
            for (int par = 0; par < 4; ++par)
                for (int l = 0; l < 64; ++l) {
                    const double* src = &wc[(size_t)(par * 4 + (l >> 4)) * cin * 16];
                    const int o = l & 15;
                    for (int k = 0; k < 4 * d.l1_ng; ++k)
                        if (k < cd) pk[((size_t)(par * d.l1_ng + k / 4) * 64 + l) * 4 + k % 4] = (float)src[(size_t)(nscore + k) * 16 + o];
                    if (nscore) sc[par * 64 + l] = (float)src[o];
                }
            if ((rc = upload(h, pk, &d.l1_wc))) return rc;
            if (nscore && (rc = upload(h, sc, &d.l1_ws))) return rc;
            std::vector<float> bc(9 * 16);
            for (int rcase = 0; rcase < 3; ++rcase)
                for (int ccase = 0; ccase < 3; ++ccase)
                    for (int o = 0; o < 16; ++o) {
                        double acc = ba[o];
                        for (int ky = 0; ky < 3; ++ky)
                            for (int kx = 0; kx < 3; ++kx) {
                                if ((rcase == 1 && ky == 0) || (rcase == 2 && ky == 2) || (ccase == 1 && kx == 0) || (ccase == 2 && kx == 2)) continue;
                                for (int m = 0; m < cout; ++m) acc += (double)wa[((size_t)o * 16 + m) * 9 + ky * 3 + kx] * (double)b[m];
                            }
                        bc[(rcase * 3 + ccase) * 16 + o] = (float)acc;
                    }
            if ((rc = upload(h, bc, &d.l1_bc))) return rc;
        }
        {
            const auto& w = h->host["conv" + n + sfx + ".0.weight"];
            const int dout = lv[j].dout, cw = deconv_width(lv[j], h->sw.pad_concat);
            const int cin = dout + lv[j].skip, cinw = cw + lv[j].skip, cout = lv[j].mid;
            if ((rc = pack_conv(h, d.conva[j], cout, 9, cinw, cinw, identity_map(cinw),
                                [&](int nn, int t, int c) {
                                    if (c >= dout && c < cw) return 0.f;
                                    const int cr = c < dout ? c : c - (cw - dout);
                                    return w[((size_t)nn * cin + cr) * 9 + t];
                                },
                                h->host["conv" + n + sfx + ".0.bias"], 3, 3))) return rc;
        }
        const auto& w2 = h->host["conv" + n + sfx + ".2.weight"];
        const auto& b2 = h->host["conv" + n + sfx + ".2.bias"];
        if (j < 5) {
            const int cin = lv[j].mid, cout = lv[j].out;
            if ((rc = pack_conv(h, d.convb[j], cout, 9, cin, cin, identity_map(cin),
                                [&](int nn, int t, int c) { return w2[((size_t)nn * cin + c) * 9 + t]; }, b2, 3, 3))) return rc;
        } else {
            const int cout = lv[j].out;
            std::vector<float> pk(9 * 16 * cout);
            for (int o = 0; o < cout; ++o)
                for (int c = 0; c < 16; ++c)
                    for (int t = 0; t < 9; ++t) pk[(t * 16 + c) * cout + o] = w2[((size_t)o * 16 + c) * 9 + t];
            if ((rc = upload(h, pk, &d.tail_w))) return rc;
            std::vector<float> pk1(9 * 16 * cout);
            for (int o = 0; o < cout; ++o)
                for (int c = 0; c < 16; ++c)
                    for (int t = 0; t < 9; ++t) pk1[(t * cout + o) * 16 + c] = w2[((size_t)o * 16 + c) * 9 + t];
            if ((rc = upload(h, pk1, &d.l1_wt))) return rc;
            for (int o = 0; o < cout; ++o) d.tail_b[o] = b2[o];
        }
    }
    return 0;
}

struct PackedHeader {
    char magic[8];
    int32_t variant, precision, circular, fuse_level1;
    char pack_group[128];
    uint64_t n_allocs, sz_encoder, sz_decoder, sz_conv;
    uint64_t n_relocs;
};
static void packed_state_io(ccvpe_handle_s* h, const std::function<void(void*, size_t)>& io) {
    io(&h->grd_enc, sizeof(EncoderW)); io(&h->sat_enc, sizeof(EncoderW));
    io(&h->grd_heads, sizeof(PackedConv)); io(&h->sat_desc, sizeof(PackedConv));
    io(h->grd_wh, sizeof(h->grd_wh)); io(h->grd_b2, sizeof(h->grd_b2));
    io(&h->loc, sizeof(DecoderW)); io(&h->ori, sizeof(DecoderW));
}

extern "C" {


int ccvpe_skip_weight(ccvpe_handle h, const char* key) {
    if (!h || !key) return ccvpe_fail(CCVPE_EINVAL, "null argument");
    if (!h->expect.count(key)) return ccvpe_fail(CCVPE_EKEY, "unexpected state_dict key '%s'", key);
    h->skipped.insert(key);
    return 0;
}

int ccvpe_set_weight(ccvpe_handle h, const char* key, const float* data, const int64_t* shape, int32_t ndim) {
    if (!h || !key || !data) return ccvpe_fail(CCVPE_EINVAL, "null argument");
    auto it = h->expect.find(key);
    if (it == h->expect.end()) return ccvpe_fail(CCVPE_EKEY, "unexpected state_dict key '%s'", key);
    const auto& es = it->second;
    bool ok = (int)es.size() == ndim;
    size_t n = 1;
    for (int i = 0; ok && i < ndim; ++i) { ok = es[i] == shape[i]; n *= (size_t)shape[i]; }
    if (!ok) return ccvpe_fail(CCVPE_EINVAL, "shape mismatch for '%s'", key);
    HIPCHK(hipSetDevice(h->cfg.device));
    std::vector<float> v(n);
    HIPCHK(hipMemcpy(v.data(), data, n * sizeof(float), hipMemcpyDefault));
    h->host[key] = std::move(v);
    h->finalized = false;
    return 0;
}

int ccvpe_finalize_weights(ccvpe_handle h) {
    if (!h) return ccvpe_fail(CCVPE_EINVAL, "null handle");
    HIPCHK(hipSetDevice(h->cfg.device));
    for (auto& kv : h->expect) {
        const std::string& k = kv.first;
        const bool optional = k.find("num_batches_tracked") != std::string::npos || k.find("._fc.") != std::string::npos;
        if (!h->host.count(k) && !(optional || h->skipped.count(k)))
            return ccvpe_fail(CCVPE_EKEY, "missing state_dict key '%s'", k.c_str());
        if (!h->host.count(k) && !optional) return ccvpe_fail(CCVPE_EKEY, "key '%s' was skipped but is required", k.c_str());
    }
    for (void* p : h->dev_allocs) (void)hipFree(p);
    h->dev_allocs.clear();
    h->dev_alloc_bytes.clear();
    h->plans.clear();
    h->last_plan = nullptr;
    int rc;
    if ((rc = build_encoder(h, h->grd_enc, "grd_efficientnet"))) return rc;
    if ((rc = build_encoder(h, h->sat_enc, "sat_efficientnet"))) return rc;
    {
        int ntot = 0;
        for (int k = 0; k < 6; ++k) ntot += h->vs.head_ch[k];
        std::vector<float> bias(ntot);
        std::vector<const std::vector<float>*> ws(6);
        std::vector<int> lvl(ntot), loc(ntot);
        int o = 0;
        for (int k = 0; k < 6; ++k) {
            std::string p = "grd_feature_to_descriptor" + std::to_string(k + 1);
            ws[k] = &h->host[p + ".0.weight"];
            const auto& b = h->host[p + ".0.bias"];
            for (int c = 0; c < h->vs.head_ch[k]; ++c, ++o) { bias[o] = b[c]; lvl[o] = k; loc[o] = c; }
            if ((rc = upload(h, h->host[p + ".2.weight"], &h->grd_wh[k]))) return rc;
            h->grd_b2[k] = h->host[p + ".2.bias"][0];
        }
        if ((rc = pack_conv(h, h->grd_heads, ntot, 1, 1280, 1280, identity_map(1280),
                            [&](int n, int, int c) { return (*ws[lvl[n]])[(size_t)loc[n] * 1280 + c]; }, bias, 1, 1))) return rc;
    }
    {
        const auto& w = h->host["sat_feature_to_descriptors.1.weight"];
        const int D = h->vs.sat_desc;
        if ((rc = pack_conv(h, h->sat_desc, D, 4, 1280, 1280, identity_map(1280),
                            [&](int n, int t, int c) { return w[(size_t)n * 5120 + c * 4 + t]; },
                            h->host["sat_feature_to_descriptors.1.bias"], 2, 2))) return rc;
    }
    if ((rc = build_decoder(h, h->loc, h->vs.loc, "", 1, true))) return rc;
    if ((rc = build_decoder(h, h->ori, h->vs.ori, "_ori", h->vs.n_rolls, false))) return rc;
    h->host.clear();
    if (!level1_supported(h->loc.l1_cxp) || !level1_supported(h->ori.l1_cxp)) h->sw.fuse_level1 = false;
    h->finalized = true;
    return 0;
}


int ccvpe_save_packed(ccvpe_handle h, const char* path) {
    if (!h || !path) return ccvpe_fail(CCVPE_EINVAL, "null argument");
    if (!h->finalized) return ccvpe_fail(CCVPE_ESTATE, "ccvpe_finalize_weights has not been called");
    static_assert(std::is_trivially_copyable<EncoderW>::value && std::is_trivially_copyable<DecoderW>::value && std::is_trivially_copyable<PackedConv>::value,
                  "descriptor structs are written as plain bytes");
    HIPCHK(hipSetDevice(h->cfg.device));
    char suffix[64];
    std::snprintf(suffix, sizeof(suffix), ".tmp.%ld.%llx", (long)getpid(), (unsigned long long)(uintptr_t)h ^ (unsigned long long)std::rand());
    const std::string tmp = std::string(path) + suffix;
    FILE* f = std::fopen(tmp.c_str(), "wb");
    if (!f) return ccvpe_fail(CCVPE_EINVAL, "cannot open %s for writing", tmp.c_str());
    std::map<uint64_t, uint64_t> index_of;
    for (size_t i = 0; i < h->dev_allocs.size(); ++i) index_of[(uint64_t)(uintptr_t)h->dev_allocs[i]] = i;
    std::vector<uint64_t> relocs;
    uint64_t word0 = 0;
    packed_state_io(h, [&](void* p, size_t n) {
        const uint64_t* w = reinterpret_cast<const uint64_t*>(p);
        for (size_t i = 0; i + 8 <= n; i += 8, ++w) {
            auto it = *w ? index_of.find(*w) : index_of.end();
            if (it != index_of.end()) { relocs.push_back(word0 + i / 8); relocs.push_back(it->second); }
        }
        word0 += n / 8;
    });
    PackedHeader hd{};
    std::memcpy(hd.magic, "CCVPEPK5", 8);
    std::snprintf(hd.pack_group, sizeof(hd.pack_group), "%s", h->sw.pack_group().c_str());
    hd.variant = h->cfg.variant; hd.precision = h->cfg.reserved[0]; hd.circular = h->cfg.circular_padding; hd.fuse_level1 = h->sw.fuse_level1 ? 1 : 0;
    hd.n_allocs = h->dev_allocs.size(); hd.sz_encoder = sizeof(EncoderW); hd.sz_decoder = sizeof(DecoderW); hd.sz_conv = sizeof(PackedConv);
    hd.n_relocs = relocs.size() / 2;
    bool ok = std::fwrite(&hd, sizeof(hd), 1, f) == 1;
    packed_state_io(h, [&](void* p, size_t n) { ok = ok && std::fwrite(p, 1, n, f) == n; });
    ok = ok && (relocs.empty() || std::fwrite(relocs.data(), 8, relocs.size(), f) == relocs.size());
    std::vector<char> buf;
    for (size_t i = 0; ok && i < h->dev_allocs.size(); ++i) {
        const uint64_t bytes = h->dev_alloc_bytes[i];
        buf.resize(bytes);
        if (hipMemcpy(buf.data(), h->dev_allocs[i], bytes, hipMemcpyDeviceToHost) != hipSuccess) { ok = false; break; }
        ok = std::fwrite(&bytes, 8, 1, f) == 1 && std::fwrite(buf.data(), 1, bytes, f) == bytes;
    }
    ok = (std::fclose(f) == 0) && ok;
    if (!ok || std::rename(tmp.c_str(), path) != 0) { std::remove(tmp.c_str()); return ccvpe_fail(CCVPE_EINVAL, "writing %s failed", path); }
    return 0;
}

int ccvpe_load_packed(ccvpe_handle h, const char* path) {
    if (!h || !path) return ccvpe_fail(CCVPE_EINVAL, "null argument");
    HIPCHK(hipSetDevice(h->cfg.device));
    FILE* f = std::fopen(path, "rb");
    if (!f) return ccvpe_fail(CCVPE_EINVAL, "cannot open %s", path);
    PackedHeader hd{};
    auto bad = [&](const char* why) { std::fclose(f); return ccvpe_fail(CCVPE_EINVAL, "%s: %s", path, why); };
    if (std::fread(&hd, sizeof(hd), 1, f) != 1 || std::memcmp(hd.magic, "CCVPEPK5", 8) != 0) return bad("not a packed-weight file of this library version");
    if (hd.variant != h->cfg.variant || hd.precision != h->cfg.reserved[0] || hd.circular != h->cfg.circular_padding) return bad("packed for a different variant / precision / padding mode");
    hd.pack_group[sizeof(hd.pack_group) - 1] = 0;
    if (h->sw.pack_group() != hd.pack_group) return bad("packed under other packer switches (CCVPE_NO_PROJ, CCVPE_WINO4_MIN_N, CCVPE_NO_WINO4, CCVPE_NO_WINO4X, CCVPE_PAD_CONCAT)");
// ... 62 lines not shown
```

ccvpe_amd/csrc/kernels.h:

```cpp
#pragma once
#include <functional>
#include <vector>
#include <hip/hip_runtime.h>
#include <stdint.h>
#include "ticket.h"

namespace ccvpe {

extern thread_local unsigned long long g_launches;
#define CCVPE_LAUNCH(...) do { ++::ccvpe::g_launches; hipLaunchKernelGGL(__VA_ARGS__); } while (0)

struct LdsAttr { size_t set[16] = {0}; };
inline void ensure_dynamic_lds(LdsAttr& state, const void* kernel, size_t bytes) {
    int dev = 0;
    if (hipGetDevice(&dev) != hipSuccess || dev < 0 || dev >= 16) dev = 0;
    if (bytes > state.set[dev] && hipFuncSetAttribute(kernel, hipFuncAttributeMaxDynamicSharedMemorySize, (int)bytes) == hipSuccess) state.set[dev] = bytes;
}

enum Act { ACT_NONE = 0, ACT_RELU = 1, ACT_SWISH = 2 };

struct Dst {
    float* ptr;
    int ld;
    int coff;
// ... 107 lines not shown
bool conv_wino4_tail_applied();
void launch_wino4x(const ConvParams& p, hipStream_t s);
bool conv_wino4x_supported(const ConvParams& p);
int conv_wino4x_config(int N);
size_t conv_wino4x_pack(int N, int cin, const std::function<float(int, int, int)>& get, std::vector<float>& out, int* cfg_out);
size_t conv_wino4_pack(int N, int cin, const std::function<float(int, int, int)>& get, std::vector<float>& out);
size_t conv_wino_pack(int N, int cin, const std::function<float(int, int, int)>& get, std::vector<float>& out, int* n16_out);
const ConvTile* conv_pw_tiles(int* n);
bool conv_pw_supported(const ConvParams& p);
bool conv_pw_fits(int bn, int kpad);
bool conv_proj_supported(const ConvParams& p, int rt);
void launch_proj(const ConvParams& p, int rt, hipStream_t s);
bool conv_proj_wanted(int N, int cin);
size_t conv_proj_pack(int N, int cin, const std::function<float(int, int)>& get, std::vector<float>& out, int taps = 1);
bool conv_proj_lat_wanted(int taps, int KH, int KW, int cinp);

struct StemParams {
    const float* in;
    int B, H, W, OH, OW;
    int pad_t, pad_l;
    int circular;
    const float* w;
    const float* bias;
    float* out;
};
void launch_stem(const StemParams& p, hipStream_t s);

struct StemDwParams {
    StemParams st;
    const float* wd;
    const float* bd;
    float* out;
    float* pool_partial;
    SeTicket se;
};
int stem_dw_tiles(int OH, int OW);
void launch_stem_dw(const StemDwParams& p, hipStream_t s);

struct DwParams {
    const float* in;
    int B, H, W, C, OH, OW;
    int k, stride, pad_t, pad_l, circular;
    const float* w;
    const float* bias;
    float* out;
    float* pool_partial;
    int S;
    SeTicket se;
};
void launch_depthwise(const DwParams& p, hipStream_t s);
int depthwise_strip_lanes(int B, int OH, int OW, int C, int k, int stride);

struct MbFrontParams {
    const float* x;
    int B, H, W, Cin, cinp;
    int mid;
    const float* we;
    const float* be;
    const float* wd;
    const float* bd;
    int k, s, pad_t, pad_l, circular, OH, OW;
    float* out;
    float* pool;
    SeTicket se;
    int spread;
};
void launch_mbconv_front(const MbFrontParams& p, hipStream_t s);
int mbconv_front_tiles(int k, int s, int OH, int OW);
int mbconv_front_ticket_rows(const MbFrontParams& p);
int mbconv_image_ticket_rows(const MbFrontParams& p);
int mbconv_front_ticket_split(const MbFrontParams& p);
bool mbconv_front_supported(int k, int s, int cin, int mid);
bool mbconv_front_profitable(int k);
bool mbconv_image_supported(const MbFrontParams& p);
int mbconv_image_strips(const MbFrontParams& p);
void launch_mbconv_image(const MbFrontParams& p, hipStream_t s);

struct SeParams {
    const float* pool_partial;
    int B, S, C, SQ;
    float inv_hw;
    const float* w1;
    const float* b1;
    const float* w2;
    const float* b2;
    float* gate;
    float* pooled;
    int SC;
    float* sq;
};
void launch_se(const SeParams& p, hipStream_t s);

struct GrdDescParams {
    const float* y;
    int B, Hf, Wf, Ntot;
    int nlev;
    int c[6], off[6];
    const float* wh[6];
    float b2[6];
    float* desc;
    int loff[6];
    int Ltot;
};
void launch_grd_desc(const GrdDescParams& p, hipStream_t s);

struct MatchParams {
    const float* x;
    int x_ld;
    int B, HW, C;
    const float* g;
    int g_ld, L;
    int R;
    int shift[32];
    uint32_t inmax;
    float* ms;
    float* cat_max;  int cat_max_ld;
    float* cat_all;  int cat_all_ld;  int rpad;
    int P;
    float* gg_scratch;
    int prep_done;
    int no_wide;
};
void launch_match(const MatchParams& p, hipStream_t s);
void launch_match_prep(const MatchParams& p, hipStream_t s);
void launch_match_prep_all(const MatchParams* ps, int n, hipStream_t s);
int match_pixels_per_block(int HW, int C);
size_t match_scratch_floats(int C);

struct TailConvParams {
    const float* in;
    int B, H, W;
    const float* w;
    float bias[2];
    int cout;
    int normalize;
    float* out;
    float* raw;
};
void launch_tail_conv(const TailConvParams& p, hipStream_t s);

struct Level1Params {
    const float* x;
    int x_ld, cx, cxp;
    int B, H, W;
    int c0, ng, score;
    const float* wc;
    const float* ws;
    const float* bc;
    const float* wt;
    float bt[2];
    int cout, normalize;
    float* out;
    float* raw;
};
void launch_level1(const Level1Params& p, hipStream_t s);
bool level1_supported(int cxp);
void launch_level1_pose(const Level1Params& p, const int* index, float* rows, hipStream_t s);
void launch_level1_topk(const Level1Params& p, const int* index, int k, float* rows, hipStream_t s);

__device__ __forceinline__ float pose_angle_deg(float cs, float sn) {
    float ang = acosf(fminf(fmaxf(cs, -1.f), 1.f)) * 57.29577951308232f;
    if (sn < 0.f) { ang = fmodf(-ang, 360.f); if (ang < 0.f) ang += 360.f; }
    return ang;
}

struct SoftmaxParams {
    const float* logits;
    int B, n;
    float* partial;
    int chunks;
    float* out;
    const float* prior;
    long long prior_stride;
};
void launch_softmax(const SoftmaxParams& p, hipStream_t s);
void launch_softmax_partial(const SoftmaxParams& p, hipStream_t s);

struct PoseArgmaxParams {
    const float* logits;
    const float* partial;
    int B, n, chunks;
    float* pairs;
    unsigned* tickets;
    int* index;
    float* rows;
    float* stats;
    const float* prior;
    long long prior_stride;
    float* posterior;
};
void launch_pose_argmax(const PoseArgmaxParams& p, hipStream_t s);
void launch_pose_gather(const float* ori, const int* index, int B, int n, float* rows, hipStream_t s);

static constexpr int TOPK_MAX_K = 64, TOPK_MAX_R = 32;
struct TopkParams {
    const float* heat;
    const float* logits;
    const float* partial;
    int B, k, r;
    unsigned long long* keys;
    unsigned* tickets;
    int* index;
    float* rows;
    const float* prior;
    long long prior_stride;
};
void launch_topk_peaks(const TopkParams& p, hipStream_t s);
void launch_topk_gather(const float* ori, const int* index, int B, int K, int n, float* rows, hipStream_t s);
size_t topk_scratch_bytes(int B);

struct PreprocParams {
    const unsigned char* in;
    int B, H, W, crop_w;
    const int* shift;
    float mean[3], stdv[3];
    float* out;
};
void launch_preprocess(const PreprocParams& p, hipStream_t s);
struct ResizeParams {
    const unsigned char* in;
    int B, IH, IW, OH, OW, crop_w;
    unsigned char* tmp;
    const int* shift;
    float mean[3], stdv[3];
    float* out;
    const int* origin;
    int map_h, map_w;
};
int launch_resize(const ResizeParams& p, hipStream_t s);

static constexpr int WARP_MAX_STAGES = 4;
static constexpr int WARP_MAX_BILINEAR = 2;
struct WarpParams {
    const unsigned char* in;
    const double* mat;
    int B, H, W, n;
    unsigned bilinear;
    int top, left, out_h, out_w;
    float mean[3], stdv[3];
    float* out;
};
int launch_warp(const WarpParams& p, hipStream_t s);

void launch_scatter_channels(const float* src, int C, long long P, Dst d0, Dst d1, int ndst, hipStream_t s);
static constexpr int GATHER_MAX_SAMPLES = 16;
struct GatherParams {
    const float* src;
    Dst d0, d1;
    int ndst;
    int C, hw;
    int b0;
    int tile[GATHER_MAX_SAMPLES];
};
void launch_gather_channels(const float* src, int C, int hw, const int* tile, int B, Dst d0, Dst d1, int ndst, hipStream_t s);

static constexpr int REGION_MAX_QUERIES = 64;
struct RegionParams {
    const float* stats;
    const float* pair_rows;
    float* rows;
    int* best_pair;
    float* tile_prob;
    int g0;
    int off[REGION_MAX_QUERIES + 1];
};
void launch_region_reduce(const float* stats, const float* pair_rows, const int* offsets, int G, float* rows, int* best_pair, float* tile_prob,
                          hipStream_t s);

static constexpr int TRACK_MAX_R = 32;
struct TrackPredictParams {
    const float* belief;
    const float* shift;
    const float* taps;
    int taps_stride;
    int radius;
    const float* floor;
    float* log_prior;
    int B;
};
void launch_track_predict(const TrackPredictParams& p, hipStream_t s);

struct PoseOut { int32_t index; float prob, cos_v, sin_v, angle_deg; };
static constexpr int PP_MAX_BATCH = 4096;
size_t postprocess_scratch_bytes(int B);
void launch_postprocess(const float* heat, const float* ori, int B, int n, PoseOut* out, float* rows, void* scratch, hipStream_t s);

struct MetricsOut { double pixel_distance, meter_distance, prob_at_gt, angle_pred_deg, angle_gt_deg, orientation_error_deg, longitudinal_m, lateral_m; };
void launch_metrics(const PoseOut* pose, const float* heat, int B, int W, int n, const int* gt_index, const float* gt_cos_sin,
                    const double* meter_per_pixel, const double* heading_deg, MetricsOut* out, hipStream_t s);

struct MultiCopy { const float* src[12]; float* dst[12]; unsigned long long n[12]; int count; };
void launch_multi_copy(const MultiCopy& mc, hipStream_t s);
void launch_fill_random(float* p, size_t n, uint32_t seed, hipStream_t s);
void launch_nhwc_to_nchw(const float* in, int in_ld, int coff, int C, int B, int HW, float* out, hipStream_t s);

}
```

ccvpe_amd/csrc/kernels_level1.hip:

```cpp
#include "kernels.h"

#include <algorithm>
#include <cstdio>

namespace ccvpe {

typedef float f32x4 __attribute__((ext_vector_type(4)));

static constexpr int T = 16;
static constexpr int AT = T + 2;
static constexpr int XT = T / 2 + 2;
static constexpr int PS = 20;
static constexpr int NPOS = (AT / 2) * (AT / 2);
static constexpr int NMT1 = (NPOS + 15) / 16;
typedef float f32x2 __attribute__((ext_vector_type(2)));


#ifndef CCVPE_L1_CLOCK
#define CCVPE_L1_CLOCK 0
#endif
#if CCVPE_L1_CLOCK
__device__ unsigned long long g_l1_clk[10];
#define CCVPE_L1_STAMP(i_) { const unsigned long long t_ = __builtin_amdgcn_s_memtime(); clk[i_] += t_ - tprev; tprev = t_; }
#else
#define CCVPE_L1_STAMP(i_)
#endif

static constexpr int KCH_MAX = 4;
static constexpr int XI_MAX = (XT * XT * KCH_MAX * 4 + 255) / 256;

static constexpr int L1_WG_PER_CU = 2;

template <int COUT, int NG, int SCORE>
__global__ __launch_bounds__(256) void level1_kernel(const Level1Params p) {
    constexpr bool POSE = false;
    const int* pose_index = nullptr;
    float* pose_rows = nullptr;
    constexpr int pose_slot = 0, pose_sample = 0, pose_ld = 0, pose_r0 = 0;
#include "kernels_level1_tile.inc"
}

template <int COUT, int NG, int SCORE>
__global__ __launch_bounds__(256) void level1_pose_kernel(const Level1Params p, const int* pose_index, float* pose_rows) {
    constexpr bool POSE = true;
    const unsigned pose_slot = blockIdx.x;
    const int pose_sample = (int)blockIdx.x;
    constexpr int pose_ld = 5, pose_r0 = 0;
#include "kernels_level1_tile.inc"
}

template <int COUT, int NG, int SCORE>
__global__ __launch_bounds__(256) void level1_topk_kernel(const Level1Params p, const int* pose_index, float* pose_rows) {
    constexpr bool POSE = true;
    const int K = (int)gridDim.x;
    const int pose_slot = (int)blockIdx.y * K + (int)blockIdx.x, pose_sample = (int)blockIdx.y;
    const int pose_ld = 5 * K, pose_r0 = 5 * (int)blockIdx.x;
    if (pose_index[pose_slot] < 0) return;
#include "kernels_level1_tile.inc"
}

bool level1_supported(int cxp) { return cxp >= 16 && cxp <= 16 * KCH_MAX && cxp % 16 == 0; }

size_t level1_lds_bytes(int cxp) {
    return ((size_t)XT * XT * (cxp + 4) + (size_t)AT * AT * PS) * sizeof(float);
}

template <typename F>
static void with_shape(const Level1Params& p, F&& f) {
    using std::integral_constant;
    if (p.ng == 10 && p.score) f(integral_constant<int, 10>{}, integral_constant<int, 1>{});
    else if (p.ng == 8 && p.score) f(integral_constant<int, 8>{}, integral_constant<int, 1>{});
    else if (p.ng == 8 && !p.score) f(integral_constant<int, 8>{}, integral_constant<int, 0>{});
    else f(integral_constant<int, 0>{}, integral_constant<int, 0>{});
}

template <int COUT, int NG, int SCORE>
static void launch_level1_t(const Level1Params& p, dim3 grid, size_t lds, hipStream_t s) {
    static LdsAttr attr;
    ensure_dynamic_lds(attr, reinterpret_cast<const void*>(level1_kernel<COUT, NG, SCORE>), lds);
    CCVPE_LAUNCH((level1_kernel<COUT, NG, SCORE>), grid, dim3(256), lds, s, p);
}

void launch_level1(const Level1Params& p, hipStream_t s) {
    const size_t lds = level1_lds_bytes(p.cxp);
    const int tiles = (p.W / T) * (p.H / T) * p.B;
    dim3 grid(std::min(tiles, L1_WG_PER_CU * 256));
#if CCVPE_L1_CLOCK
    static int calls = 0;
    const bool stamp = ++calls % 4 == 0;
    if (stamp) { (void)hipStreamSynchronize(s); unsigned long long z[10] = {}; (void)hipMemcpyToSymbol(HIP_SYMBOL(g_l1_clk), z, sizeof z); }
#endif
    if (p.cout == 1) with_shape(p, [&](auto ng, auto sc) { launch_level1_t<1, decltype(ng)::value, decltype(sc)::value>(p, grid, lds, s); });
    else with_shape(p, [&](auto ng, auto sc) { launch_level1_t<2, decltype(ng)::value, decltype(sc)::value>(p, grid, lds, s); });
#if CCVPE_L1_CLOCK
    if (stamp) {
        (void)hipStreamSynchronize(s);
        unsigned long long h[10];
        (void)hipMemcpyFromSymbol(h, HIP_SYMBOL(g_l1_clk), sizeof h);
        double tot = 0;
        for (int i = 0; i < 5; ++i) tot += (double)h[i];
        std::fprintf(stderr, "level1<%d> cx %d: %.0f cycles/tile and wave: input->LDS+barrier %.0f %% conv_a %.0f %% tail products %.0f %% barrier %.0f %% tail conv %.0f %%\n",
                     p.cout, p.cx, tot / std::max(1.0, (double)h[8]), 100 * h[0] / tot, 100 * h[1] / tot, 100 * h[2] / tot, 100 * h[3] / tot, 100 * h[4] / tot);
    }
#endif
}

void launch_level1_pose(const Level1Params& p, const int* index, float* rows, hipStream_t s) {
    const size_t lds = level1_lds_bytes(p.cxp);
    with_shape(p, [&](auto ng, auto sc) {
        constexpr int NG = decltype(ng)::value, SCORE = decltype(sc)::value;
        static LdsAttr attr;
        ensure_dynamic_lds(attr, reinterpret_cast<const void*>(level1_pose_kernel<2, NG, SCORE>), lds);
        CCVPE_LAUNCH((level1_pose_kernel<2, NG, SCORE>), dim3(p.B), dim3(256), lds, s, p, index, rows);
    });
}

void launch_level1_topk(const Level1Params& p, const int* index, int k, float* rows, hipStream_t s) {
    const size_t lds = level1_lds_bytes(p.cxp);
    with_shape(p, [&](auto ng, auto sc) {
        constexpr int NG = decltype(ng)::value, SCORE = decltype(sc)::value;
        static LdsAttr attr;
        ensure_dynamic_lds(attr, reinterpret_cast<const void*>(level1_topk_kernel<2, NG, SCORE>), lds);
        CCVPE_LAUNCH((level1_topk_kernel<2, NG, SCORE>), dim3(k, p.B), dim3(256), lds, s, p, index, rows);
    });
}

}
```

ccvpe_amd/csrc/kernels_level1_tile.inc:

```
extern __shared__ __attribute__((aligned(16))) float smem[];
const int CXP = p.cxp;
const int XS = CXP + 4;
float* Xs = smem;
float* Ps = smem + XT * XT * XS;

const int tid = threadIdx.x, lane = tid & 63, wave = tid >> 6;
const int H = p.H, W = p.W;
const int IH = H >> 1, IW = W >> 1;
const int tiles_x = W / T, tiles_y = H / T;
const int tiles = p.B * tiles_x * tiles_y;
const int xcd = blockIdx.x & 7;
const int stride = ((int)gridDim.x >> 3) + (xcd < ((int)gridDim.x & 7) ? 1 : 0);
const int t_begin = xcd * (tiles >> 3) + min(xcd, tiles & 7);
int t_end = t_begin + (tiles >> 3) + (xcd < (tiles & 7) ? 1 : 0);
int tile = t_begin + ((int)blockIdx.x >> 3);
int pose_pix = 0;
if constexpr (POSE) {
    pose_pix = min(max(pose_index[pose_slot], 0), H * W - 1);
    tile = pose_sample * (tiles_x * tiles_y) + (pose_pix / W / T) * tiles_x + (pose_pix % W) / T;
    t_end = tile + 1;
}
if (tile >= t_end) return;

constexpr int NPT = (9 * COUT + 15) / 16;
f32x4 wtf[NPT];
#pragma unroll
for (int nt = 0; nt < NPT; ++nt) {
    const int n = nt * 16 + (lane & 15);
    wtf[nt] = n < 9 * COUT ? *reinterpret_cast<const f32x4*>(p.wt + (size_t)n * 16 + 4 * (lane >> 4)) : f32x4{0.f, 0.f, 0.f, 0.f};
}
constexpr bool NG_RT = NG == 0;
constexpr int NGR = NG_RT ? 16 : NG;
const int ng = NG_RT ? p.ng : NG;
const bool score = NG_RT ? p.score != 0 : SCORE != 0;
const float wsc = score ? p.ws[wave * 64 + lane] : 0.f;
f32x4 wg[NGR];
#pragma unroll
for (int g = 0; g < NGR; ++g)
    wg[g] = g < ng ? *reinterpret_cast<const f32x4*>(p.wc + ((size_t)(wave * ng + g) * 64 + lane) * 4) : f32x4{0.f, 0.f, 0.f, 0.f};
const f32x4 bint = *reinterpret_cast<const f32x4*>(p.bc + 4 * (lane >> 4));
const int py = wave >> 1, px = wave & 1;
int xoff[NMT1], pq[NMT1];
#pragma unroll
for (int mt = 0; mt < NMT1; ++mt) {
    const int pos = min(mt * 16 + (lane & 15), NPOS - 1);
    const int i = pos / 9, j = pos % 9;
    xoff[mt] = ((i + ((lane >> 4) >> 1)) * XT + j + ((lane >> 4) & 1)) * XS + p.c0;
    pq[mt] = mt * 16 + (lane & 15) < NPOS ? (2 * i + 1 - py) * AT + 2 * j + 1 - px : -1;
}

const int c4n = CXP >> 2;
const __amdgpu_buffer_rsrc_t x_rsrc = __builtin_amdgcn_make_buffer_rsrc(const_cast<float*>(p.x), 0, (unsigned)((size_t)p.B * IH * IW * p.x_ld * 4), 0x00020000);
int x_lds[XI_MAX], x_rc[XI_MAX];
#pragma unroll
for (int it = 0; it < XI_MAX; ++it) {
    const int i = tid + it * 256;
    const int px_ = i / c4n, c4 = i - px_ * c4n;
    const bool live = i < XT * XT * c4n;
    x_lds[it] = live ? px_ * XS + c4 * 4 : -1;
    x_rc[it] = ((px_ / XT) << 8) | (px_ % XT) | ((c4 * 4 < p.cx ? c4 * 4 : 0x7fff) << 16);
}
f32x4 xv[XI_MAX];
#define CCVPE_L1_LOAD_X(tl)                                                                              \
{                                                                                                    \
    const int b_ = (tl) / (tiles_x * tiles_y);                                                       \
    const int r_ = (tl) - b_ * (tiles_x * tiles_y);                                                  \
    const int ty_ = r_ / tiles_x, tx_ = r_ - ty_ * tiles_x;                                          \
    const int xr0_ = ty_ * (T / 2) - 1, xc0_ = tx_ * (T / 2) - 1;                                    \
    _Pragma("unroll") for (int it = 0; it < XI_MAX; ++it) {                                          \
        const int xr = xr0_ + ((x_rc[it] >> 8) & 0xff), xc = xc0_ + (x_rc[it] & 0xff), ch = x_rc[it] >> 16; \
        const bool ok = x_lds[it] >= 0 && (unsigned)xr < (unsigned)IH && (unsigned)xc < (unsigned)IW && ch != 0x7fff; \
        const unsigned off = ok ? (unsigned)((((b_ * IH + xr) * IW + xc) * p.x_ld + ch) * 4) : 0x80000000u; \
        xv[it] = __builtin_bit_cast(f32x4, __builtin_amdgcn_raw_buffer_load_b128(x_rsrc, off, 0, 0)); \
    }                                                                                                \
}
CCVPE_L1_LOAD_X(tile);

const int oy = tid >> 4, ox = tid & 15;
const size_t hw = (size_t)H * W;

#if CCVPE_L1_CLOCK
unsigned long long clk[7] = {0, 0, 0, 0, 0, 0, 0}, tprev = __builtin_amdgcn_s_memtime();
int ntiles = 0;
#endif
while (true) {
#if CCVPE_L1_CLOCK
    ++ntiles;
#endif
    const int b = tile / (tiles_x * tiles_y);
    const int rem = tile - b * (tiles_x * tiles_y);
    const int Y0 = (rem / tiles_x) * T, X0 = (rem % tiles_x) * T;
    const bool interior = Y0 >= 2 && Y0 + T + 2 <= H && X0 >= 2 && X0 + T + 2 <= W;

#pragma unroll
    for (int it = 0; it < XI_MAX; ++it)
        if (x_lds[it] >= 0) *reinterpret_cast<f32x4*>(Xs + x_lds[it]) = xv[it];
    __syncthreads();
    CCVPE_L1_STAMP(0);
    const int tile_n = tile + stride;
    const bool have_n = tile_n < t_end;
    if (have_n) { CCVPE_L1_LOAD_X(tile_n); }

    f32x4 acc[NMT1];
#pragma unroll
    for (int mt = 0; mt < NMT1; ++mt) acc[mt] = f32x4{0.f, 0.f, 0.f, 0.f};
    if (score) {
#pragma unroll
        for (int mt = 0; mt < NMT1; ++mt) acc[mt] = __builtin_amdgcn_mfma_f32_16x16x4f32(wsc, Xs[xoff[mt] - p.c0], acc[mt], 0, 0, 0);
    }
#pragma unroll
    for (int g = 0; g < NGR; ++g) {
        if (!NG_RT || g < ng) {
            f32x4 a[NMT1];
#pragma unroll
            for (int mt = 0; mt < NMT1; ++mt) a[mt] = *reinterpret_cast<const f32x4*>(Xs + xoff[mt] + 4 * g);
#pragma unroll
            for (int e = 0; e < 4; ++e)
#pragma unroll
                for (int mt = 0; mt < NMT1; ++mt) acc[mt] = __builtin_amdgcn_mfma_f32_16x16x4f32(wg[g][e], a[mt][e], acc[mt], 0, 0, 0);
        }
    }
    CCVPE_L1_STAMP(1);

#pragma unroll
    for (int mt = 0; mt < NMT1; ++mt) {
        const int q = max(pq[mt], 0);
        f32x4 v;
        if (interior) {
            v = acc[mt] + bint;
        } else {
            const int gy = Y0 - 1 + q / AT, gx = X0 - 1 + q % AT;
            const int bcase = (gy == 0 ? 3 : gy == H - 1 ? 6 : 0) + (gx == 0 ? 1 : gx == W - 1 ? 2 : 0);
            v = acc[mt] + *reinterpret_cast<const f32x4*>(p.bc + bcase * 16 + 4 * (lane >> 4));
            if (!((unsigned)gy < (unsigned)H && (unsigned)gx < (unsigned)W)) v = f32x4{0.f, 0.f, 0.f, 0.f};
        }
#pragma unroll
        for (int r = 0; r < 4; ++r) v[r] = fmaxf(v[r], 0.f);
#pragma unroll
        for (int nt = 0; nt < NPT; ++nt) {
            f32x4 pa = {0.f, 0.f, 0.f, 0.f};
#pragma unroll
            for (int e = 0; e < 4; ++e) pa = __builtin_amdgcn_mfma_f32_16x16x4f32(wtf[nt][e], v[e], pa, 0, 0, 0);
            if (pq[mt] >= 0) {
                if (nt == 0) *reinterpret_cast<f32x4*>(Ps + q * PS + 4 * (lane >> 4)) = pa;
                else if ((lane >> 4) == 0) *reinterpret_cast<f32x2*>(Ps + q * PS + 16) = f32x2{pa[0], pa[1]};
            }
        }
    }
    CCVPE_L1_STAMP(2);
    __syncthreads();
    CCVPE_L1_STAMP(3);

    float o[COUT];
#pragma unroll
    for (int c = 0; c < COUT; ++c) o[c] = p.bt[c];
#pragma unroll
    for (int t = 0; t < 9; ++t) {
        const float* pp = Ps + ((oy + t / 3) * AT + ox + t % 3) * PS + t * COUT;
        if (COUT == 2) { const f32x2 v = *reinterpret_cast<const f32x2*>(pp); o[0] += v.x; o[COUT - 1] += v.y; }
        else o[0] += pp[0];
    }
    const size_t opix = (size_t)(Y0 + oy) * W + X0 + ox;
    if (p.raw) {
#pragma unroll
        for (int c = 0; c < COUT; ++c) p.raw[((size_t)b * COUT + c) * hw + opix] = o[c];
    }
    if (p.normalize) {
        float n2 = 0.f;
#pragma unroll
        for (int c = 0; c < COUT; ++c) n2 = fmaf(o[c], o[c], n2);
        const float inv = 1.f / fmaxf(sqrtf(n2), 1e-12f);
#pragma unroll
        for (int c = 0; c < COUT; ++c) o[c] *= inv;
    }
    if constexpr (POSE) {
        static_assert(COUT == 2, "the pose form serves the orientation decoder");
        if (opix == (size_t)pose_pix) {
            pose_rows[b * pose_ld + pose_r0 + 2] = o[0];
            pose_rows[b * pose_ld + pose_r0 + 3] = o[1];
            pose_rows[b * pose_ld + pose_r0 + 4] = pose_angle_deg(o[0], o[1]);
        }
        break;
    }
#pragma unroll
    for (int c = 0; c < COUT; ++c) p.out[((size_t)b * COUT + c) * hw + opix] = o[c];

    CCVPE_L1_STAMP(4);
    if (!have_n) break;
    tile = tile_n;
}
#if CCVPE_L1_CLOCK
if (lane == 0) {
    for (int i = 0; i < 7; ++i) atomicAdd(&g_l1_clk[i], clk[i]);
    atomicAdd(&g_l1_clk[7], 1ull);
    atomicAdd(&g_l1_clk[8], (unsigned long long)ntiles);
}
#endif
#undef CCVPE_L1_LOAD_X
```

include/ccvpe.h:

```cpp
#ifndef CCVPE_H
#define CCVPE_H

#include <stddef.h>
#include <stdint.h>

#ifdef __cplusplus
extern "C" {
#endif

#define CCVPE_OK 0
#define CCVPE_EINVAL (-1)
#define CCVPE_ESTATE (-2)
#define CCVPE_EHIP (-3)
#define CCVPE_ENOMEM (-4)
#define CCVPE_EKEY (-5)

#define CCVPE_VARIANT_VIGOR 0
#define CCVPE_VARIANT_VIGOR_ORI_PRIOR 1
#define CCVPE_VARIANT_KITTI 2
#define CCVPE_VARIANT_OXFORD 3

#define CCVPE_OUT_HW 512
#define CCVPE_SAT_HW 512

// ... 11 lines not shown
typedef struct ccvpe_outputs {
    float* logits_flattened;
    float* heatmap;
    float* ori;
    float* matching_score[6];
} ccvpe_outputs;

typedef struct ccvpe_pose {
    int32_t index;
    float   prob;
    float   cos_v, sin_v;
    float   angle_deg;
} ccvpe_pose;

typedef struct ccvpe_metrics {
    double pixel_distance;
    double meter_distance;
    double prob_at_gt;
    double angle_pred_deg;
    double angle_gt_deg;
    double orientation_error_deg;
    double longitudinal_m;
    double lateral_m;
} ccvpe_metrics;

const char* ccvpe_last_error(void);
const char* ccvpe_version(void);
uint64_t ccvpe_launch_count(void);

int ccvpe_create(const ccvpe_config* cfg, ccvpe_handle* out);
int ccvpe_destroy(ccvpe_handle h);

int ccvpe_set_weight(ccvpe_handle h, const char* key, const float* data, const int64_t* shape, int32_t ndim);
int ccvpe_skip_weight(ccvpe_handle h, const char* key);
int ccvpe_finalize_weights(ccvpe_handle h);

int ccvpe_save_packed(ccvpe_handle h, const char* path);
int ccvpe_load_packed(ccvpe_handle h, const char* path);
const char* ccvpe_pack_switches(void);

int ccvpe_import_tuning(ccvpe_handle h, const char* text);
int ccvpe_export_tuning(ccvpe_handle h, char* buf, size_t capacity, size_t* needed);
int ccvpe_tuning_generation(ccvpe_handle h);

int ccvpe_max_micro_batch(int32_t variant, float ori_noise, int32_t grd_h, int32_t grd_w);

int ccvpe_output_channels(ccvpe_handle h, int32_t level);
size_t ccvpe_workspace_bytes(ccvpe_handle h, int32_t batch, int32_t grd_h, int32_t grd_w);

int ccvpe_forward(ccvpe_handle h, const float* grd, int32_t grd_h, int32_t grd_w, const float* sat,
                  int32_t batch, const ccvpe_outputs* out, void* stream);

int ccvpe_postprocess(ccvpe_handle h, const float* heatmap, const float* ori, int32_t batch,
                      ccvpe_pose* poses, void* stream);
int ccvpe_postprocess_rows(ccvpe_handle h, const float* heatmap, const float* ori, int32_t batch,
                           float* rows, void* stream);
int ccvpe_postprocess_topk(ccvpe_handle h, const float* heatmap, const float* ori, int32_t batch, int32_t k,
                           int32_t radius, float* rows, void* stream);

int ccvpe_eval_metrics(ccvpe_handle h, const ccvpe_pose* poses, const float* heatmap, int32_t batch, const int32_t* gt_index,
                       const float* gt_cos_sin, const double* meter_per_pixel, const double* heading_deg, ccvpe_metrics* out,
                       void* stream);

size_t ccvpe_aerial_cache_bytes(ccvpe_handle h, int32_t batch);
int ccvpe_encode_aerial(ccvpe_handle h, const float* sat, int32_t batch, void* cache, void* stream);
int ccvpe_forward_cached(ccvpe_handle h, const float* grd, int32_t grd_h, int32_t grd_w, const void* cache,
                         int32_t batch, const ccvpe_outputs* out, void* stream);

int ccvpe_localize(ccvpe_handle h, const float* grd, int32_t grd_h, int32_t grd_w, const float* sat,
                   int32_t batch, float* rows, void* stream);
int ccvpe_localize_cached(ccvpe_handle h, const float* grd, int32_t grd_h, int32_t grd_w, const void* cache,
                          int32_t batch, float* rows, void* stream);
int ccvpe_localize_topk(ccvpe_handle h, const float* grd, int32_t grd_h, int32_t grd_w, const float* sat,
                        int32_t batch, int32_t k, int32_t radius, float* rows, void* stream);
int ccvpe_localize_topk_cached(ccvpe_handle h, const float* grd, int32_t grd_h, int32_t grd_w, const void* cache,
                               int32_t batch, int32_t k, int32_t radius, float* rows, void* stream);

int ccvpe_forward_cached_indexed(ccvpe_handle h, const float* grd, int32_t grd_h, int32_t grd_w, const void* cache,
                                 int32_t n_tiles, const int32_t* tile_index, int32_t batch, const ccvpe_outputs* out,
                                 void* stream);
int ccvpe_localize_cached_indexed(ccvpe_handle h, const float* grd, int32_t grd_h, int32_t grd_w, const void* cache,
                                  int32_t n_tiles, const int32_t* tile_index, int32_t batch, float* rows, void* stream);
int ccvpe_localize_topk_cached_indexed(ccvpe_handle h, const float* grd, int32_t grd_h, int32_t grd_w, const void* cache,
                                       int32_t n_tiles, const int32_t* tile_index, int32_t batch, int32_t k, int32_t radius,
                                       float* rows, void* stream);

size_t ccvpe_ground_cache_bytes(ccvpe_handle h, int32_t batch, int32_t grd_h, int32_t grd_w);
int ccvpe_encode_ground(ccvpe_handle h, const float* grd, int32_t grd_h, int32_t grd_w, int32_t batch, void* cache,
                        void* stream);

int ccvpe_localize_region(ccvpe_handle h, const void* grd_cache, int32_t n_queries, int32_t grd_h, int32_t grd_w,
                          const void* sat_cache, int32_t n_tiles, const int32_t* offsets, const int32_t* tiles,
                          float* rows, int32_t* best_pair, float* pair_rows, float* pair_stats, float* tile_prob,
                          void* stream);

int ccvpe_localize_prior(ccvpe_handle h, const float* grd, int32_t grd_h, int32_t grd_w, const float* sat, int32_t batch,
                         const float* log_prior, int64_t prior_stride, int32_t k, int32_t radius, float* rows, void* stream);
int ccvpe_localize_prior_cached_indexed(ccvpe_handle h, const float* grd, int32_t grd_h, int32_t grd_w, const void* cache,
                                        int32_t n_tiles, const int32_t* tile_index, int32_t batch, const float* log_prior,
                                        int64_t prior_stride, int32_t k, int32_t radius, float* rows, void* stream);
int ccvpe_postprocess_prior(ccvpe_handle h, const float* logits, const float* ori, int32_t batch, const float* log_prior,
                            int64_t prior_stride, int32_t k, int32_t radius, float* rows, void* stream);
int ccvpe_localize_region_prior(ccvpe_handle h, const void* grd_cache, int32_t n_queries, int32_t grd_h, int32_t grd_w,
                                const void* sat_cache, int32_t n_tiles, const int32_t* offsets, const int32_t* tiles,
                                const float* pair_log_prior, int64_t prior_stride, float* rows, int32_t* best_pair,
                                float* pair_rows, float* pair_stats, float* tile_prob, void* stream);

int ccvpe_track_update(ccvpe_handle h, const float* grd, int32_t grd_h, int32_t grd_w, const float* sat, int32_t batch,
                       const float* log_prior, int64_t prior_stride, float* rows, float* posterior, void* stream);
int ccvpe_track_update_cached_indexed(ccvpe_handle h, const float* grd, int32_t grd_h, int32_t grd_w, const void* cache,
                                      int32_t n_tiles, const int32_t* tile_index, int32_t batch, const float* log_prior,
                                      int64_t prior_stride, float* rows, float* posterior, void* stream);
int ccvpe_track_update_logits(ccvpe_handle h, const float* logits, const float* ori, int32_t batch, const float* log_prior,
                              int64_t prior_stride, float* rows, float* posterior, void* stream);
int ccvpe_track_predict(ccvpe_handle h, const float* belief, int32_t batch, const float* shift, const float* taps,
                        int32_t taps_stride, int32_t radius, const float* floor, float* log_prior, void* stream);

int ccvpe_preprocess(const uint8_t* hwc, int32_t batch, int32_t H, int32_t W, const int32_t* shift, int32_t crop_w,
                     const float mean[3], const float stdv[3], float* out_nchw, void* stream);

int ccvpe_preprocess_resize(const uint8_t* hwc, int32_t batch, int32_t in_h, int32_t in_w, int32_t out_h, int32_t out_w,
                            const int32_t* shift, int32_t crop_w, const float mean[3], const float stdv[3], uint8_t* scratch,
                            float* out_nchw, void* stream);

#define CCVPE_RESAMPLE_NEAREST 0
#define CCVPE_RESAMPLE_BILINEAR 2
int ccvpe_preprocess_affine(const uint8_t* hwc, int32_t batch, int32_t H, int32_t W, const double* matrices, const int32_t* filters,
                            int32_t n_stages, int32_t top, int32_t left, int32_t out_h, int32_t out_w, const float mean[3],
                            const float stdv[3], float* out_nchw, void* stream);

int ccvpe_preprocess_window_resize(const uint8_t* map_hwc, int32_t map_h, int32_t map_w, const int32_t* origins, int32_t batch,
                                   int32_t win_h, int32_t win_w, int32_t out_h, int32_t out_w, const float mean[3], const float stdv[3],
                                   uint8_t* scratch, float* out_nchw, void* stream);

int ccvpe_set_debug(ccvpe_handle h, int32_t enable);
int ccvpe_set_streams(ccvpe_handle h, int32_t n_streams);
int ccvpe_read_tap(ccvpe_handle h, const char* name, float* host_dst, size_t capacity, size_t* n_out,
                   int32_t shape_out[4]);

int ccvpe_debug_dump_plan(ccvpe_handle h, const char* path);

int ccvpe_profile_forward(ccvpe_handle h, const float* grd, int32_t grd_h, int32_t grd_w, const float* sat,
                          int32_t batch, const ccvpe_outputs* out, void* stream);
int ccvpe_profile_row(ccvpe_handle h, int32_t i, char* name_buf, size_t name_cap, float* ms,
                      double* flops, double* bytes);
int ccvpe_profile_row_issued(ccvpe_handle h, int32_t i, double* issued_flops);

int ccvpe_op_num_tiles(void);
const char* ccvpe_op_tile_name(int32_t tile);
int ccvpe_op_conv2d(const float* in, int32_t B, int32_t H, int32_t W, int32_t Cin, const float* w, const float* bias,
                    int32_t Cout, int32_t KH, int32_t KW, int32_t stride, int32_t pad, int32_t act, int32_t tile,
                    float* out, int32_t iters, float* ms, void* stream);

#ifdef __cplusplus
}
#endif
#endif
```

Measured before the change: 2593 queries/s.

## Add 16x32 tile variant for fused level-1 decoder kernel and a standalone op entry

```diff
diff --git a/ccvpe_amd/_lib.py b/ccvpe_amd/_lib.py
--- a/ccvpe_amd/_lib.py
+++ b/ccvpe_amd/_lib.py
@@ -114,6 +114,8 @@
     ("ccvpe_op_conv2d", C.c_int, [C.c_void_p, C.c_int32, C.c_int32, C.c_int32, C.c_int32, C.c_void_p, C.c_void_p,
                                   C.c_int32, C.c_int32, C.c_int32, C.c_int32, C.c_int32, C.c_int32, C.c_int32,
                                   C.c_void_p, C.c_int32, C.POINTER(C.c_float), C.c_void_p]),
+    ("ccvpe_op_level1", C.c_int, [C.c_void_p, C.c_int32, C.c_int32, C.c_int32, C.c_int32, C.c_int32, C.c_void_p, C.c_void_p,
+                                  C.c_void_p, C.c_void_p, C.c_void_p, C.c_void_p, C.c_int32, C.c_int32, C.c_void_p, C.c_void_p]),
 ]
 
 
@@ -229,6 +231,25 @@
                              C.c_void_p(out.data_ptr()), iters, C.byref(ms), C.c_void_p(stream))
     check(rc, "ccvpe_op_conv2d")
     return out, (ms.value if iters > 0 else None)
+
+
+def op_level1(x_nhwc, wd, bd, wa, ba, wt, bt, score=False, tile=1, max_wg=0):
+    import torch
+    lib = load()
+    B, h, w, Cin = x_nhwc.shape
+    Cout = wt.shape[0]
+    x = x_nhwc.float()
+    if score:
+        x = torch.cat([x[..., :1], x.new_zeros((B, h, w, 7)), x[..., 1:]], dim=-1)
+    x = x.contiguous()
+    ws = [t.detach().float().contiguous() for t in (wd, bd, wa, ba, wt, bt)]
+    out = torch.empty((B, Cout, 2 * h, 2 * w), dtype=torch.float32, device=x.device)
+    stream = torch.cuda.current_stream(x.device).cuda_stream
+    rc = lib.ccvpe_op_level1(C.c_void_p(x.data_ptr()), B, 2 * h, 2 * w, Cin, 1 if score else 0, *[C.c_void_p(t.data_ptr()) for t in ws],
+                             Cout, tile | (max_wg << 8), C.c_void_p(out.data_ptr()), C.c_void_p(stream))
+    check(rc, "ccvpe_op_level1")
+    return out, rc
+
 
 _lib = None
 
diff --git a/ccvpe_amd/csrc/ccvpe_api.hip b/ccvpe_amd/csrc/ccvpe_api.hip
--- a/ccvpe_amd/csrc/ccvpe_api.hip
+++ b/ccvpe_amd/csrc/ccvpe_api.hip
@@ -28,6 +28,7 @@
     if (const char* e = getenv("CCVPE_AUTOTUNE")) s.autotune = std::atoi(e) != 0;
     if (const char* e = getenv("CCVPE_FUSE_MBCONV")) s.fuse_mbconv = std::atoi(e);
     if (const char* e = getenv("CCVPE_FUSE_L1")) s.fuse_level1 = std::atoi(e) != 0;
+    if (const char* e = getenv("CCVPE_L1_TILE")) s.l1_tile = std::atoi(e);
     if (const char* e = getenv("CCVPE_WINOGRAD")) s.wino = std::atoi(e) != 0;
     if (const char* e = getenv("CCVPE_GRAPH")) s.graph_mode = std::atoi(e) != 0;
     if (const char* e = getenv("CCVPE_STREAMS")) s.two_streams = std::atoi(e) >= 2;
@@ -1115,4 +1116,40 @@
     return 0;
 }
 
-}
+int ccvpe_op_level1(const float* in, int32_t B, int32_t H, int32_t W, int32_t Cin, int32_t score, const float* wd, const float* bd,
+                    const float* wa, const float* ba, const float* wt, const float* bt, int32_t Cout, int32_t tile, float* out, void* stream) {
+    if (!in || !wd || !bd || !wa || !ba || !wt || !bt || !out) return ccvpe_fail(CCVPE_EINVAL, "null argument");
+    const int cd = Cin - (score ? 1 : 0);
+    if (B <= 0 || H <= 0 || W <= 0 || H % 16 || W % 16 || (Cout != 1 && Cout != 2) || cd <= 0 || cd % 4 || tile < 0 || (tile & 0xff) > 1 || ((tile >> 8) != 0 && (tile >> 8) < 8))
+        return ccvpe_fail(CCVPE_EINVAL, "bad level-1 geometry (H, W multiples of 16, Cout 1 or 2, descriptor channels a multiple of 4, tile 0 or 1, workgroup cap 0 or >= 8)");
+    if ((double)B * H * W * 16 >= 2147483647.0) return ccvpe_fail(CCVPE_EINVAL, "tensor exceeds 2^31 elements");
+    std::vector<float> hwd((size_t)Cin * 64), hbd(16), hwa(16 * 16 * 9), hba(16), hwt((size_t)Cout * 16 * 9), hbt(Cout);
+    HIPCHK(hipMemcpy(hwd.data(), wd, hwd.size() * sizeof(float), hipMemcpyDefault));
+    HIPCHK(hipMemcpy(hbd.data(), bd, hbd.size() * sizeof(float), hipMemcpyDefault));
+    HIPCHK(hipMemcpy(hwa.data(), wa, hwa.size() * sizeof(float), hipMemcpyDefault));
+    HIPCHK(hipMemcpy(hba.data(), ba, hba.size() * sizeof(float), hipMemcpyDefault));
+    HIPCHK(hipMemcpy(hwt.data(), wt, hwt.size() * sizeof(float), hipMemcpyDefault));
+    HIPCHK(hipMemcpy(hbt.data(), bt, hbt.size() * sizeof(float), hipMemcpyDefault));
+    ccvpe_handle_s tmp;
+    DecoderW d;
+    auto cleanup = [&]() { for (void* p : tmp.dev_allocs) (void)hipFree(p); };
+    int rc = compose_level1(&tmp, d, hwd, hbd, hwa, hba, Cin, score ? 1 : 0);
+    if (!rc) rc = pack_level1_tail(&tmp, d, hwt, hbt, Cout);
+    if (rc) { cleanup(); return rc; }
+    if (!level1_supported(d.l1_cxp)) { cleanup(); return ccvpe_fail(CCVPE_EINVAL, "the fused level takes up to 64 input channels"); }
+    Level1Params lp{};
+    lp.x = in; lp.x_ld = d.l1_cx; lp.cx = d.l1_cx; lp.cxp = d.l1_cxp; lp.B = B; lp.H = H; lp.W = W;
+    lp.c0 = d.l1_c0; lp.ng = d.l1_ng; lp.score = d.l1_score; lp.wc = d.l1_wc; lp.ws = d.l1_ws; lp.bc = d.l1_bc; lp.wt = d.l1_wt;
+    lp.bt[0] = d.tail_b[0]; lp.bt[1] = d.tail_b[1]; lp.cout = Cout; lp.normalize = Cout == 2 ? 1 : 0;
+    lp.out = out; lp.raw = nullptr; lp.tile = tile & 0xff; lp.max_wg = tile >> 8;
+    hipStream_t st = (hipStream_t)stream;
+    launch_level1(lp, st);
+    hipError_t e = hipGetLastError();
+    hipError_t e2 = hipStreamSynchronize(st);
+    cleanup();
+    if (e != hipSuccess) return ccvpe_fail(CCVPE_EHIP, "level-1 launch failed: %s", hipGetErrorString(e));
+    if (e2 != hipSuccess) return ccvpe_fail(CCVPE_EHIP, "level-1 execution failed: %s", hipGetErrorString(e2));
+    return level1_tile(lp);
+}
+
+}
diff --git a/ccvpe_amd/csrc/ccvpe_internal.h b/ccvpe_amd/csrc/ccvpe_internal.h
--- a/ccvpe_amd/csrc/ccvpe_internal.h
+++ b/ccvpe_amd/csrc/ccvpe_internal.h
@@ -99,6 +99,7 @@
     bool autotune = true;
     int fuse_mbconv = 1;
     bool fuse_level1 = true;
+    int l1_tile = 1;
     bool wino = true;
     int graph_mode = 0;
     bool two_streams = true;
@@ -184,6 +185,10 @@
     float *l1_wc = nullptr, *l1_ws = nullptr, *l1_bc = nullptr;
     int l1_cx = 0, l1_cxp = 0, l1_c0 = 0, l1_ng = 0, l1_score = 0;
 };
+struct ccvpe_handle_s;
+int compose_level1(ccvpe_handle_s* h, DecoderW& d, const std::vector<float>& w, const std::vector<float>& b, const std::vector<float>& wa,
+                   const std::vector<float>& ba, int cin, int nscore);
+int pack_level1_tail(ccvpe_handle_s* h, DecoderW& d, const std::vector<float>& w2, const std::vector<float>& b2, int cout);
 
 struct Tensor {
     int id = -1; int B = 0, H = 0, W = 0, C = 0;
diff --git a/ccvpe_amd/csrc/ccvpe_plan.hip b/ccvpe_amd/csrc/ccvpe_plan.hip
--- a/ccvpe_amd/csrc/ccvpe_plan.hip
+++ b/ccvpe_amd/csrc/ccvpe_plan.hip
@@ -434,6 +434,7 @@
         lp.x_ld = din.C; lp.cx = dw.l1_cx; lp.cxp = dw.l1_cxp; lp.B = B; lp.H = CCVPE_OUT_HW; lp.W = CCVPE_OUT_HW;
         lp.c0 = dw.l1_c0; lp.ng = dw.l1_ng; lp.score = dw.l1_score; lp.wc = dw.l1_wc; lp.ws = dw.l1_ws; lp.bc = dw.l1_bc; lp.wt = dw.l1_wt;
         lp.bt[0] = dw.tail_b[0]; lp.bt[1] = dw.tail_b[1]; lp.cout = cout; lp.normalize = is_ori ? 1 : 0;
+        lp.tile = h->sw.l1_tile;
         const bool has_raw = raw.id >= 0;
         std::vector<Tensor> uses = {din};
         if (has_raw) uses.push_back(raw);
diff --git a/ccvpe_amd/csrc/ccvpe_weights.hip b/ccvpe_amd/csrc/ccvpe_weights.hip
--- a/ccvpe_amd/csrc/ccvpe_weights.hip
+++ b/ccvpe_amd/csrc/ccvpe_weights.hip
@@ -204,6 +204,68 @@
     return pack_pointwise_bn(h, e.head, p + "._conv_head.weight", p + "._bn1", 1280, 320);
 }
 
+
+int compose_level1(ccvpe_handle_s* h, DecoderW& d, const std::vector<float>& w, const std::vector<float>& b, const std::vector<float>& wa,
+                   const std::vector<float>& ba, int cin, int nscore) {
+    int rc;
+    const int cout = 16;
+    const int spad = score_pad(nscore);
+    const int cd = cin - nscore;
+    d.l1_cx = spad + cd;
+    d.l1_cxp = round_up(d.l1_cx, 16);
+    d.l1_c0 = spad; d.l1_ng = (cd + 3) / 4; d.l1_score = nscore;
+    std::vector<double> wc((size_t)16 * cin * 16, 0.0);
+    for (int py = 0; py < 2; ++py)
+        for (int px = 0; px < 2; ++px)
+            for (int ky = 0; ky < 3; ++ky)
+                for (int kx = 0; kx < 3; ++kx) {
+                    const int ty = py + ky + 1, tx = px + kx + 1, a = (ty >> 1) - py, bb = (tx >> 1) - px;
+                    const int qd = (ty & 1) * 2 + (tx & 1);
+                    double* dst = &wc[(size_t)(((py * 2 + px) * 2 + a) * 2 + bb) * cin * 16];
+                    for (int c = 0; c < cin; ++c)
+                        for (int o = 0; o < 16; ++o) {
+                            double acc = 0.0;
+                            for (int m = 0; m < cout; ++m)
+                                acc += (double)wa[((size_t)o * 16 + m) * 9 + ky * 3 + kx] * (double)w[((size_t)c * cout + m) * 4 + qd];
+                            dst[(size_t)c * 16 + o] += acc;
+                        }
+                }
+    std::vector<float> pk((size_t)4 * d.l1_ng * 64 * 4, 0.f), sc(4 * 64, 0.f);
+    for (int par = 0; par < 4; ++par)
+        for (int l = 0; l < 64; ++l) {
+            const double* src = &wc[(size_t)(par * 4 + (l >> 4)) * cin * 16];
+            const int o = l & 15;
+            for (int k = 0; k < 4 * d.l1_ng; ++k)
+                if (k < cd) pk[((size_t)(par * d.l1_ng + k / 4) * 64 + l) * 4 + k % 4] = (float)src[(size_t)(nscore + k) * 16 + o];
+            if (nscore) sc[par * 64 + l] = (float)src[o];
+        }
+    if ((rc = upload(h, pk, &d.l1_wc))) return rc;
+    if (nscore && (rc = upload(h, sc, &d.l1_ws))) return rc;
+    std::vector<float> bc(9 * 16);
+    for (int rcase = 0; rcase < 3; ++rcase)
+        for (int ccase = 0; ccase < 3; ++ccase)
+            for (int o = 0; o < 16; ++o) {
+                double acc = ba[o];
+                for (int ky = 0; ky < 3; ++ky)
+                    for (int kx = 0; kx < 3; ++kx) {
+                        if ((rcase == 1 && ky == 0) || (rcase == 2 && ky == 2) || (ccase == 1 && kx == 0) || (ccase == 2 && kx == 2)) continue;
+                        for (int m = 0; m < cout; ++m) acc += (double)wa[((size_t)o * 16 + m) * 9 + ky * 3 + kx] * (double)b[m];
+                    }
+                bc[(rcase * 3 + ccase) * 16 + o] = (float)acc;
+            }
+    if ((rc = upload(h, bc, &d.l1_bc))) return rc;
+    return 0;
+}
+
+int pack_level1_tail(ccvpe_handle_s* h, DecoderW& d, const std::vector<float>& w2, const std::vector<float>& b2, int cout) {
+    std::vector<float> pk1(9 * 16 * cout);
+    for (int o = 0; o < cout; ++o)
+        for (int c = 0; c < 16; ++c)
+            for (int t = 0; t < 9; ++t) pk1[(t * cout + o) * 16 + c] = w2[((size_t)o * 16 + c) * 9 + t];
+    if (int rc = upload(h, pk1, &d.l1_wt)) return rc;
+    for (int o = 0; o < cout; ++o) d.tail_b[o] = b2[o];
+    return 0;
+}
 
 static int build_decoder(ccvpe_handle_s* h, DecoderW& d, const DecLevel* lv, const std::string& sfx, int nscore_l6, bool every_level_scored) {
     int rc;
@@ -227,57 +289,8 @@
                                 bias, 1, 1))) return rc;
         }
         if (j == 5) {
-            const auto& w = h->host["deconv" + n + sfx + ".weight"];
-            const auto& b = h->host["deconv" + n + sfx + ".bias"];
-            const auto& wa = h->host["conv" + n + sfx + ".0.weight"];
-            const auto& ba = h->host["conv" + n + sfx + ".0.bias"];
-            const int cin = lv[j].din, cout = lv[j].dout;
-            const int nscore = every_level_scored ? 1 : 0;
-            const int spad = score_pad(nscore);
-            const int cd = cin - nscore;
-            d.l1_cx = spad + cd;
-            d.l1_cxp = round_up(d.l1_cx, 16);
-            d.l1_c0 = spad; d.l1_ng = (cd + 3) / 4; d.l1_score = nscore;
-            std::vector<double> wc((size_t)16 * cin * 16, 0.0);
-            for (int py = 0; py < 2; ++py)
-                for (int px = 0; px < 2; ++px)
-                    for (int ky = 0; ky < 3; ++ky)
-                        for (int kx = 0; kx < 3; ++kx) {
-                            const int ty = py + ky + 1, tx = px + kx + 1, a = (ty >> 1) - py, bb = (tx >> 1) - px;
-                            const int qd = (ty & 1) * 2 + (tx & 1);
-                            double* dst = &wc[(size_t)(((py * 2 + px) * 2 + a) * 2 + bb) * cin * 16];
-                            for (int c = 0; c < cin; ++c)
-                                for (int o = 0; o < 16; ++o) {
-                                    double acc = 0.0;
-                                    for (int m = 0; m < cout; ++m)
-                                        acc += (double)wa[((size_t)o * 16 + m) * 9 + ky * 3 + kx] * (double)w[((size_t)c * cout + m) * 4 + qd];
-                                    dst[(size_t)c * 16 + o] += acc;
-                                }
-                        }
-            std::vector<float> pk((size_t)4 * d.l1_ng * 64 * 4, 0.f), sc(4 * 64, 0.f);
-            for (int par = 0; par < 4; ++par)
-                for (int l = 0; l < 64; ++l) {
-                    const double* src = &wc[(size_t)(par * 4 + (l >> 4)) * cin * 16];
-                    const int o = l & 15;
-                    for (int k = 0; k < 4 * d.l1_ng; ++k)
-                        if (k < cd) pk[((size_t)(par * d.l1_ng + k / 4) * 64 + l) * 4 + k % 4] = (float)src[(size_t)(nscore + k) * 16 + o];
-                    if (nscore) sc[par * 64 + l] = (float)src[o];
-                }
-            if ((rc = upload(h, pk, &d.l1_wc))) return rc;
-            if (nscore && (rc = upload(h, sc, &d.l1_ws))) return rc;
-            std::vector<float> bc(9 * 16);
-            for (int rcase = 0; rcase < 3; ++rcase)
-                for (int ccase = 0; ccase < 3; ++ccase)
-                    for (int o = 0; o < 16; ++o) {
-                        double acc = ba[o];
-                        for (int ky = 0; ky < 3; ++ky)
-                            for (int kx = 0; kx < 3; ++kx) {
-                                if ((rcase == 1 && ky == 0) || (rcase == 2 && ky == 2) || (ccase == 1 && kx == 0) || (ccase == 2 && kx == 2)) continue;
-                                for (int m = 0; m < cout; ++m) acc += (double)wa[((size_t)o * 16 + m) * 9 + ky * 3 + kx] * (double)b[m];
-                            }
-                        bc[(rcase * 3 + ccase) * 16 + o] = (float)acc;
-                    }
-            if ((rc = upload(h, bc, &d.l1_bc))) return rc;
+            if ((rc = compose_level1(h, d, h->host["deconv" + n + sfx + ".weight"], h->host["deconv" + n + sfx + ".bias"], h->host["conv" + n + sfx + ".0.weight"],
+                                     h->host["conv" + n + sfx + ".0.bias"], lv[j].din, every_level_scored ? 1 : 0))) return rc;
         }
         {
             const auto& w = h->host["conv" + n + sfx + ".0.weight"];
@@ -304,12 +317,7 @@
                 for (int c = 0; c < 16; ++c)
                     for (int t = 0; t < 9; ++t) pk[(t * 16 + c) * cout + o] = w2[((size_t)o * 16 + c) * 9 + t];
             if ((rc = upload(h, pk, &d.tail_w))) return rc;
-            std::vector<float> pk1(9 * 16 * cout);
-            for (int o = 0; o < cout; ++o)
-                for (int c = 0; c < 16; ++c)
-                    for (int t = 0; t < 9; ++t) pk1[(t * cout + o) * 16 + c] = w2[((size_t)o * 16 + c) * 9 + t];
-            if ((rc = upload(h, pk1, &d.l1_wt))) return rc;
-            for (int o = 0; o < cout; ++o) d.tail_b[o] = b2[o];
+            if ((rc = pack_level1_tail(h, d, w2, b2, cout))) return rc;
         }
     }
     return 0;
diff --git a/ccvpe_amd/csrc/kernels.h b/ccvpe_amd/csrc/kernels.h
--- a/ccvpe_amd/csrc/kernels.h
+++ b/ccvpe_amd/csrc/kernels.h
@@ -283,8 +283,11 @@
     int cout, normalize;
     float* out;
     float* raw;
+    int tile;
+    int max_wg;
 };
 void launch_level1(const Level1Params& p, hipStream_t s);
+int level1_tile(const Level1Params& p);
 bool level1_supported(int cxp);
 void launch_level1_pose(const Level1Params& p, const int* index, float* rows, hipStream_t s);
 void launch_level1_topk(const Level1Params& p, const int* index, int k, float* rows, hipStream_t s);
diff --git a/ccvpe_amd/csrc/kernels_level1.hip b/ccvpe_amd/csrc/kernels_level1.hip
--- a/ccvpe_amd/csrc/kernels_level1.hip
+++ b/ccvpe_amd/csrc/kernels_level1.hip
@@ -7,13 +7,13 @@
 
 typedef float f32x4 __attribute__((ext_vector_type(4)));
 
-static constexpr int T = 16;
-static constexpr int AT = T + 2;
-static constexpr int XT = T / 2 + 2;
-static constexpr int PS = 20;
-static constexpr int NPOS = (AT / 2) * (AT / 2);
-static constexpr int NMT1 = (NPOS + 15) / 16;
 typedef float f32x2 __attribute__((ext_vector_type(2)));
+
+template <int TILE> struct L1Shape;
+template <> struct L1Shape<0> { static constexpr int TY = 16, TX = 16, NTHR = 256; };
+template <> struct L1Shape<1> { static constexpr int TY = 16, TX = 32, NTHR = 512; };
+static constexpr int L1_TILES = 2;
+static constexpr int l1_ps(int cout, int tx) { return tx == 16 ? 20 : 9 * cout; }
 
 
 #ifndef CCVPE_L1_CLOCK
@@ -27,12 +27,11 @@
 #endif
 
 static constexpr int KCH_MAX = 4;
-static constexpr int XI_MAX = (XT * XT * KCH_MAX * 4 + 255) / 256;
 
-static constexpr int L1_WG_PER_CU = 2;
+static constexpr int L1_WAVES_PER_CU = 8;
 
-template <int COUT, int NG, int SCORE>
-__global__ __launch_bounds__(256) void level1_kernel(const Level1Params p) {
+template <int COUT, int NG, int SCORE, int TILE>
+__global__ __launch_bounds__(L1Shape<TILE>::NTHR) void level1_kernel(const Level1Params p) {
     constexpr bool POSE = false;
     const int* pose_index = nullptr;
     float* pose_rows = nullptr;
@@ -43,6 +42,7 @@
 template <int COUT, int NG, int SCORE>
 __global__ __launch_bounds__(256) void level1_pose_kernel(const Level1Params p, const int* pose_index, float* pose_rows) {
     constexpr bool POSE = true;
+    constexpr int TILE = 0;
     const unsigned pose_slot = blockIdx.x;
     const int pose_sample = (int)blockIdx.x;
     constexpr int pose_ld = 5, pose_r0 = 0;
@@ -52,6 +52,7 @@
 template <int COUT, int NG, int SCORE>
 __global__ __launch_bounds__(256) void level1_topk_kernel(const Level1Params p, const int* pose_index, float* pose_rows) {
     constexpr bool POSE = true;
+    constexpr int TILE = 0;
     const int K = (int)gridDim.x;
     const int pose_slot = (int)blockIdx.y * K + (int)blockIdx.x, pose_sample = (int)blockIdx.y;
     const int pose_ld = 5 * K, pose_r0 = 5 * (int)blockIdx.x;
@@ -61,8 +62,15 @@
 
 bool level1_supported(int cxp) { return cxp >= 16 && cxp <= 16 * KCH_MAX && cxp % 16 == 0; }
 
-size_t level1_lds_bytes(int cxp) {
-    return ((size_t)XT * XT * (cxp + 4) + (size_t)AT * AT * PS) * sizeof(float);
+template <int TILE>
+static size_t lds_bytes(int cxp, int cout) {
+    using S = L1Shape<TILE>;
+    return ((size_t)(S::TY / 2 + 2) * (S::TX / 2 + 2) * (cxp + 4) + (size_t)(S::TY + 2) * (S::TX + 2) * l1_ps(cout, S::TX)) * sizeof(float);
+}
+
+int level1_tile(const Level1Params& p) {
+    const int t = p.tile < 0 || p.tile >= L1_TILES ? 0 : p.tile;
+    return t == 1 && (p.H % L1Shape<1>::TY || p.W % L1Shape<1>::TX) ? 0 : t;
 }
 
 template <typename F>
@@ -74,24 +82,34 @@
     else f(integral_constant<int, 0>{}, integral_constant<int, 0>{});
 }
 
-template <int COUT, int NG, int SCORE>
-static void launch_level1_t(const Level1Params& p, dim3 grid, size_t lds, hipStream_t s) {
+template <int COUT, int NG, int SCORE, int TILE>
+static void launch_level1_t(const Level1Params& p, hipStream_t s) {
+    using S = L1Shape<TILE>;
+    const size_t lds = lds_bytes<TILE>(p.cxp, COUT);
+    const int tiles = (p.W / S::TX) * (p.H / S::TY) * p.B;
+    dim3 grid(std::min(tiles, p.max_wg >= 8 ? p.max_wg : L1_WAVES_PER_CU * 64 / S::NTHR * 256));
     static LdsAttr attr;
-    ensure_dynamic_lds(attr, reinterpret_cast<const void*>(level1_kernel<COUT, NG, SCORE>), lds);
-    CCVPE_LAUNCH((level1_kernel<COUT, NG, SCORE>), grid, dim3(256), lds, s, p);
+    ensure_dynamic_lds(attr, reinterpret_cast<const void*>(level1_kernel<COUT, NG, SCORE, TILE>), lds);
+    CCVPE_LAUNCH((level1_kernel<COUT, NG, SCORE, TILE>), grid, dim3(S::NTHR), lds, s, p);
+}
+
+template <int COUT>
+static void launch_level1_c(const Level1Params& p, hipStream_t s) {
+    with_shape(p, [&](auto ng, auto sc) {
+        constexpr int NG = decltype(ng)::value, SCORE = decltype(sc)::value;
+        if (level1_tile(p) == 1) launch_level1_t<COUT, NG, SCORE, 1>(p, s);
+        else launch_level1_t<COUT, NG, SCORE, 0>(p, s);
+    });
 }
 
 void launch_level1(const Level1Params& p, hipStream_t s) {
-    const size_t lds = level1_lds_bytes(p.cxp);
-    const int tiles = (p.W / T) * (p.H / T) * p.B;
-    dim3 grid(std::min(tiles, L1_WG_PER_CU * 256));
 #if CCVPE_L1_CLOCK
     static int calls = 0;
     const bool stamp = ++calls % 4 == 0;
     if (stamp) { (void)hipStreamSynchronize(s); unsigned long long z[10] = {}; (void)hipMemcpyToSymbol(HIP_SYMBOL(g_l1_clk), z, sizeof z); }
 #endif
-    if (p.cout == 1) with_shape(p, [&](auto ng, auto sc) { launch_level1_t<1, decltype(ng)::value, decltype(sc)::value>(p, grid, lds, s); });
-    else with_shape(p, [&](auto ng, auto sc) { launch_level1_t<2, decltype(ng)::value, decltype(sc)::value>(p, grid, lds, s); });
+    if (p.cout == 1) launch_level1_c<1>(p, s);
+    else launch_level1_c<2>(p, s);
 #if CCVPE_L1_CLOCK
     if (stamp) {
         (void)hipStreamSynchronize(s);
@@ -106,7 +124,7 @@
 }
 
 void launch_level1_pose(const Level1Params& p, const int* index, float* rows, hipStream_t s) {
-    const size_t lds = level1_lds_bytes(p.cxp);
+    const size_t lds = lds_bytes<0>(p.cxp, 2);
     with_shape(p, [&](auto ng, auto sc) {
         constexpr int NG = decltype(ng)::value, SCORE = decltype(sc)::value;
         static LdsAttr attr;
@@ -116,7 +134,7 @@
 }
 
 void launch_level1_topk(const Level1Params& p, const int* index, int k, float* rows, hipStream_t s) {
-    const size_t lds = level1_lds_bytes(p.cxp);
+    const size_t lds = lds_bytes<0>(p.cxp, 2);
     with_shape(p, [&](auto ng, auto sc) {
         constexpr int NG = decltype(ng)::value, SCORE = decltype(sc)::value;
         static LdsAttr attr;
diff --git a/ccvpe_amd/csrc/kernels_level1_tile.inc b/ccvpe_amd/csrc/kernels_level1_tile.inc
--- a/ccvpe_amd/csrc/kernels_level1_tile.inc
+++ b/ccvpe_amd/csrc/kernels_level1_tile.inc
@@ -1,13 +1,21 @@
+constexpr int TY = L1Shape<TILE>::TY, TX = L1Shape<TILE>::TX, NTHR = L1Shape<TILE>::NTHR;
+constexpr int ATY = TY + 2, ATX = TX + 2;
+constexpr int XTY = TY / 2 + 2, XTX = TX / 2 + 2;
+constexpr int PS = l1_ps(COUT, TX);
+constexpr int NPX = ATX / 2, NPOS = (ATY / 2) * NPX;
+constexpr int NPART = NTHR / 256;
+constexpr int NMT1 = ((NPOS + 15) / 16 + NPART - 1) / NPART;
+constexpr int XI_MAX = (XTY * XTX * KCH_MAX * 4 + NTHR - 1) / NTHR;
 extern __shared__ __attribute__((aligned(16))) float smem[];
 const int CXP = p.cxp;
 const int XS = CXP + 4;
 float* Xs = smem;
-float* Ps = smem + XT * XT * XS;
+float* Ps = smem + XTY * XTX * XS;
 
 const int tid = threadIdx.x, lane = tid & 63, wave = tid >> 6;
 const int H = p.H, W = p.W;
 const int IH = H >> 1, IW = W >> 1;
-const int tiles_x = W / T, tiles_y = H / T;
+const int tiles_x = W / TX, tiles_y = H / TY;
 const int tiles = p.B * tiles_x * tiles_y;
 const int xcd = blockIdx.x & 7;
 const int stride = ((int)gridDim.x >> 3) + (xcd < ((int)gridDim.x & 7) ? 1 : 0);
@@ -17,7 +25,7 @@
 int pose_pix = 0;
 if constexpr (POSE) {
     pose_pix = min(max(pose_index[pose_slot], 0), H * W - 1);
-    tile = pose_sample * (tiles_x * tiles_y) + (pose_pix / W / T) * tiles_x + (pose_pix % W) / T;
+    tile = pose_sample * (tiles_x * tiles_y) + (pose_pix / W / TY) * tiles_x + (pose_pix % W) / TX;
     t_end = tile + 1;
 }
 if (tile >= t_end) return;
@@ -33,20 +41,22 @@
 constexpr int NGR = NG_RT ? 16 : NG;
 const int ng = NG_RT ? p.ng : NG;
 const bool score = NG_RT ? p.score != 0 : SCORE != 0;
-const float wsc = score ? p.ws[wave * 64 + lane] : 0.f;
+const int cls = wave & 3, part = wave >> 2;
+const float wsc = score ? p.ws[cls * 64 + lane] : 0.f;
 f32x4 wg[NGR];
 #pragma unroll
 for (int g = 0; g < NGR; ++g)
-    wg[g] = g < ng ? *reinterpret_cast<const f32x4*>(p.wc + ((size_t)(wave * ng + g) * 64 + lane) * 4) : f32x4{0.f, 0.f, 0.f, 0.f};
+    wg[g] = g < ng ? *reinterpret_cast<const f32x4*>(p.wc + ((size_t)(cls * ng + g) * 64 + lane) * 4) : f32x4{0.f, 0.f, 0.f, 0.f};
 const f32x4 bint = *reinterpret_cast<const f32x4*>(p.bc + 4 * (lane >> 4));
-const int py = wave >> 1, px = wave & 1;
+const int py = cls >> 1, px = cls & 1;
 int xoff[NMT1], pq[NMT1];
 #pragma unroll
 for (int mt = 0; mt < NMT1; ++mt) {
-    const int pos = min(mt * 16 + (lane & 15), NPOS - 1);
-    const int i = pos / 9, j = pos % 9;
-    xoff[mt] = ((i + ((lane >> 4) >> 1)) * XT + j + ((lane >> 4) & 1)) * XS + p.c0;
-    pq[mt] = mt * 16 + (lane & 15) < NPOS ? (2 * i + 1 - py) * AT + 2 * j + 1 - px : -1;
+    const int row = (part * NMT1 + mt) * 16 + (lane & 15);
+    const int pos = min(row, NPOS - 1);
+    const int i = pos / NPX, j = pos % NPX;
+    xoff[mt] = ((i + ((lane >> 4) >> 1)) * XTX + j + ((lane >> 4) & 1)) * XS + p.c0;
+    pq[mt] = row < NPOS ? (2 * i + 1 - py) * ATX + 2 * j + 1 - px : -1;
 }
 
 const int c4n = CXP >> 2;
@@ -54,11 +64,11 @@
 int x_lds[XI_MAX], x_rc[XI_MAX];
 #pragma unroll
 for (int it = 0; it < XI_MAX; ++it) {
-    const int i = tid + it * 256;
+    const int i = tid + it * NTHR;
     const int px_ = i / c4n, c4 = i - px_ * c4n;
-    const bool live = i < XT * XT * c4n;
+    const bool live = i < XTY * XTX * c4n;
     x_lds[it] = live ? px_ * XS + c4 * 4 : -1;
-    x_rc[it] = ((px_ / XT) << 8) | (px_ % XT) | ((c4 * 4 < p.cx ? c4 * 4 : 0x7fff) << 16);
+    x_rc[it] = ((px_ / XTX) << 8) | (px_ % XTX) | ((c4 * 4 < p.cx ? c4 * 4 : 0x7fff) << 16);
 }
 f32x4 xv[XI_MAX];
 #define CCVPE_L1_LOAD_X(tl)                                                                              \
@@ -66,7 +76,7 @@
     const int b_ = (tl) / (tiles_x * tiles_y);                                                       \
     const int r_ = (tl) - b_ * (tiles_x * tiles_y);                                                  \
     const int ty_ = r_ / tiles_x, tx_ = r_ - ty_ * tiles_x;                                          \
-    const int xr0_ = ty_ * (T / 2) - 1, xc0_ = tx_ * (T / 2) - 1;                                    \
+    const int xr0_ = ty_ * (TY / 2) - 1, xc0_ = tx_ * (TX / 2) - 1;                                   \
     _Pragma("unroll") for (int it = 0; it < XI_MAX; ++it) {                                          \
         const int xr = xr0_ + ((x_rc[it] >> 8) & 0xff), xc = xc0_ + (x_rc[it] & 0xff), ch = x_rc[it] >> 16; \
         const bool ok = x_lds[it] >= 0 && (unsigned)xr < (unsigned)IH && (unsigned)xc < (unsigned)IW && ch != 0x7fff; \
@@ -76,7 +86,6 @@
 }
 CCVPE_L1_LOAD_X(tile);
 
-const int oy = tid >> 4, ox = tid & 15;
 const size_t hw = (size_t)H * W;
 
 #if CCVPE_L1_CLOCK
@@ -89,8 +98,8 @@
 #endif
     const int b = tile / (tiles_x * tiles_y);
     const int rem = tile - b * (tiles_x * tiles_y);
-    const int Y0 = (rem / tiles_x) * T, X0 = (rem % tiles_x) * T;
-    const bool interior = Y0 >= 2 && Y0 + T + 2 <= H && X0 >= 2 && X0 + T + 2 <= W;
+    const int Y0 = (rem / tiles_x) * TY, X0 = (rem % tiles_x) * TX;
+    const bool interior = Y0 >= 2 && Y0 + TY + 2 <= H && X0 >= 2 && X0 + TX + 2 <= W;
 
 #pragma unroll
     for (int it = 0; it < XI_MAX; ++it)
@@ -129,7 +138,7 @@
         if (interior) {
             v = acc[mt] + bint;
         } else {
-            const int gy = Y0 - 1 + q / AT, gx = X0 - 1 + q % AT;
+            const int gy = Y0 - 1 + q / ATX, gx = X0 - 1 + q % ATX;
             const int bcase = (gy == 0 ? 3 : gy == H - 1 ? 6 : 0) + (gx == 0 ? 1 : gx == W - 1 ? 2 : 0);
             v = acc[mt] + *reinterpret_cast<const f32x4*>(p.bc + bcase * 16 + 4 * (lane >> 4));
             if (!((unsigned)gy < (unsigned)H && (unsigned)gx < (unsigned)W)) v = f32x4{0.f, 0.f, 0.f, 0.f};
@@ -142,8 +151,19 @@
 #pragma unroll
             for (int e = 0; e < 4; ++e) pa = __builtin_amdgcn_mfma_f32_16x16x4f32(wtf[nt][e], v[e], pa, 0, 0, 0);
             if (pq[mt] >= 0) {
-                if (nt == 0) *reinterpret_cast<f32x4*>(Ps + q * PS + 4 * (lane >> 4)) = pa;
-                else if ((lane >> 4) == 0) *reinterpret_cast<f32x2*>(Ps + q * PS + 16) = f32x2{pa[0], pa[1]};
+                float* pd = Ps + q * PS + 4 * (lane >> 4);
+                if (nt == 0) {
+                    if constexpr (PS % 4 == 0) {
+                        *reinterpret_cast<f32x4*>(pd) = pa;
+                    } else if constexpr (PS % 2 == 0) {
+                        *reinterpret_cast<f32x2*>(pd) = f32x2{pa[0], pa[1]};
+                        *reinterpret_cast<f32x2*>(pd + 2) = f32x2{pa[2], pa[3]};
+                    } else {
+#pragma unroll
+                        for (int e = 0; e < 4; ++e)
+                            if (4 * (lane >> 4) + e < 9 * COUT) pd[e] = pa[e];
+                    }
+                } else if ((lane >> 4) == 0) *reinterpret_cast<f32x2*>(Ps + q * PS + 16) = f32x2{pa[0], pa[1]};
             }
         }
     }
@@ -151,39 +171,44 @@
     __syncthreads();
     CCVPE_L1_STAMP(3);
 
-    float o[COUT];
-#pragma unroll
-    for (int c = 0; c < COUT; ++c) o[c] = p.bt[c];
-#pragma unroll
-    for (int t = 0; t < 9; ++t) {
-        const float* pp = Ps + ((oy + t / 3) * AT + ox + t % 3) * PS + t * COUT;
-        if (COUT == 2) { const f32x2 v = *reinterpret_cast<const f32x2*>(pp); o[0] += v.x; o[COUT - 1] += v.y; }
-        else o[0] += pp[0];
-    }
-    const size_t opix = (size_t)(Y0 + oy) * W + X0 + ox;
-    if (p.raw) {
-#pragma unroll
-        for (int c = 0; c < COUT; ++c) p.raw[((size_t)b * COUT + c) * hw + opix] = o[c];
-    }
-    if (p.normalize) {
-        float n2 = 0.f;
-#pragma unroll
-        for (int c = 0; c < COUT; ++c) n2 = fmaf(o[c], o[c], n2);
-        const float inv = 1.f / fmaxf(sqrtf(n2), 1e-12f);
-#pragma unroll
-        for (int c = 0; c < COUT; ++c) o[c] *= inv;
-    }
-    if constexpr (POSE) {
-        static_assert(COUT == 2, "the pose form serves the orientation decoder");
-        if (opix == (size_t)pose_pix) {
-            pose_rows[b * pose_ld + pose_r0 + 2] = o[0];
-            pose_rows[b * pose_ld + pose_r0 + 3] = o[1];
-            pose_rows[b * pose_ld + pose_r0 + 4] = pose_angle_deg(o[0], o[1]);
-        }
-        break;
-    }
-#pragma unroll
-    for (int c = 0; c < COUT; ++c) p.out[((size_t)b * COUT + c) * hw + opix] = o[c];
+#pragma unroll
+    for (int r = 0; r < TY * TX / NTHR; ++r) {
+        const int oy = (tid + r * NTHR) / TX, ox = (tid + r * NTHR) % TX;
+        float o[COUT];
+#pragma unroll
+        for (int c = 0; c < COUT; ++c) o[c] = p.bt[c];
+#pragma unroll
+        for (int t = 0; t < 9; ++t) {
+            const float* pp = Ps + ((oy + t / 3) * ATX + ox + t % 3) * PS + t * COUT;
+            if (COUT == 2) { const f32x2 v = *reinterpret_cast<const f32x2*>(pp); o[0] += v.x; o[COUT - 1] += v.y; }
+            else o[0] += pp[0];
+        }
+        const size_t opix = (size_t)(Y0 + oy) * W + X0 + ox;
+        if (p.raw) {
+#pragma unroll
+            for (int c = 0; c < COUT; ++c) p.raw[((size_t)b * COUT + c) * hw + opix] = o[c];
+        }
+        if (p.normalize) {
+            float n2 = 0.f;
+#pragma unroll
+            for (int c = 0; c < COUT; ++c) n2 = fmaf(o[c], o[c], n2);
+            const float inv = 1.f / fmaxf(sqrtf(n2), 1e-12f);
+#pragma unroll
+            for (int c = 0; c < COUT; ++c) o[c] *= inv;
+        }
+        if constexpr (POSE) {
+            static_assert(COUT == 2, "the pose form serves the orientation decoder");
+            if (opix == (size_t)pose_pix) {
+                pose_rows[b * pose_ld + pose_r0 + 2] = o[0];
+                pose_rows[b * pose_ld + pose_r0 + 3] = o[1];
+                pose_rows[b * pose_ld + pose_r0 + 4] = pose_angle_deg(o[0], o[1]);
+            }
+        } else {
+#pragma unroll
+            for (int c = 0; c < COUT; ++c) p.out[((size_t)b * COUT + c) * hw + opix] = o[c];
+        }
+    }
+    if constexpr (POSE) break;
 
     CCVPE_L1_STAMP(4);
     if (!have_n) break;
diff --git a/include/ccvpe.h b/include/ccvpe.h
--- a/include/ccvpe.h
+++ b/include/ccvpe.h
@@ -187,6 +187,9 @@
                     int32_t Cout, int32_t KH, int32_t KW, int32_t stride, int32_t pad, int32_t act, int32_t tile,
                     float* out, int32_t iters, float* ms, void* stream);
 
+int ccvpe_op_level1(const float* in, int32_t B, int32_t H, int32_t W, int32_t Cin, int32_t score, const float* wd, const float* bd,
+                    const float* wa, const float* ba, const float* wt, const float* bt, int32_t Cout, int32_t tile, float* out, void* stream);
+
 #ifdef __cplusplus
 }
 #endif
```

Result: faster. 2629 queries/s (median of 6 runs) (+1.4%).
